# maruchitatsuki/python-based-Sequential-Monte-Carlo-method-with-likelihood-tempering

Measured on AMD Instinct MI355X. Metric: particle-mutation-steps/sec, higher is better.
Workload: dtype f64

## Files before the change

include/smc_hip.h:

```cpp
#ifndef SMC_HIP_H
#define SMC_HIP_H

#include <stddef.h>
#include <stdint.h>

#ifdef __cplusplus
extern "C" {
#endif

#define SMC_ABI_VERSION 3
#define SMC_MAX_DIM 8
#define SMC_MAX_ESS_CAND 16
#define SMC_MAX_RANKS 64

#define SMC_SET_PRED 0
#define SMC_SET_FILT 1

#define SMC_PRIOR_UNIFORM 0
#define SMC_PRIOR_NORMAL 1
#define SMC_PRIOR_FLAT 2
#define SMC_PRIOR_LOGNORMAL 3
#define SMC_PRIOR_GAMMA 4
#define SMC_PRIOR_BETA 5
#define SMC_PRIOR_TRUNCNORMAL 6
// ... 96 lines not shown
int smc_user_model_check4(const char *source, int n_states, int dim, int method, int n_obs, int proportional, char *log, int log_cap);
int smc_user_model_dump_source4(const char *source, int n_states, int dim, int method, int n_obs, int proportional, const char *dir);
int smc_set_model_user5(smc_ctx *ctx, const char *source, int n_states, int n_obs, const double *t, const double *obs,
                        const double *cond, const double *obs_scale, int n_ex, int n_t, int n_cond, const int *add_index,
                        const double *add_fixed, const int *prop_index, const double *prop_fixed, double rtol, double atol, int method,
                        int est_sigma, double sigma_fixed, const double *in_t, const double *in_u, int n_in, int n_knot);
int smc_user_model_check5(const char *source, int n_states, int dim, int method, int n_obs, int noise, int n_cond, int n_in, int n_knot,
                          char *log, int log_cap);
int smc_user_model_dump_source5(const char *source, int n_states, int dim, int method, int n_obs, int noise, int n_cond, int n_in,
                                int n_knot, const char *dir);
int smc_set_model_user6(smc_ctx *ctx, const char *source, int n_states, int n_obs, const double *t, const double *obs,
                        const double *cond, const double *obs_scale, int n_ex, int n_t, int n_cond, const int *add_index,
                        const double *add_fixed, const int *prop_index, const double *prop_fixed, double rtol, double atol, int method,
                        int est_sigma, double sigma_fixed, const double *in_t, const double *in_u, int n_in, int n_knot,
                        const double *ev_t, const double *ev_v, int n_ev, int n_val);
int smc_user_model_check6(const char *source, int n_states, int dim, int method, int n_obs, int noise, int n_cond, int n_in, int n_knot,
                          int n_ev, int n_val, char *log, int log_cap);
int smc_user_model_dump_source6(const char *source, int n_states, int dim, int method, int n_obs, int noise, int n_cond, int n_in,
                                int n_knot, int n_ev, int n_val, const char *dir);
int smc_set_model_user7(smc_ctx *ctx, const char *source, int n_states, int n_obs, const double *t, const double *obs,
                        const double *cond, const double *obs_scale, int n_ex, int n_t, int n_cond, const int *add_index,
                        const double *add_fixed, const int *prop_index, const double *prop_fixed, double rtol, double atol, int method,
                        int est_sigma, double sigma_fixed, const double *in_t, const double *in_u, int n_in, int n_knot,
                        const double *ev_t, const double *ev_v, int n_ev, int n_val, const signed char *censor);
int smc_user_model_check7(const char *source, int n_states, int dim, int method, int n_obs, int noise, int n_cond, int n_in, int n_knot,
                          int n_ev, int n_val, int censor, char *log, int log_cap);
int smc_user_model_dump_source7(const char *source, int n_states, int dim, int method, int n_obs, int noise, int n_cond, int n_in,
                                int n_knot, int n_ev, int n_val, int censor, const char *dir);
int smc_user_predict(smc_ctx *ctx, const double *particle, int64_t n, double *lk, double *pred, int64_t *n_failed, int64_t *attempts);
int smc_user_predict_at(smc_ctx *ctx, const double *particle, int64_t n, const double *t_new, const double *cond_new, int n_ex_new,
                        int n_t_new, double *pred, int64_t *n_failed, int64_t *attempts);
#define SMC_PRED_NOISE_GAUSSIAN 1
#define SMC_PRED_NOISE_FAMILY 2
int smc_user_predict_summary(smc_ctx *ctx, int set, const double *t_new, const double *cond_new, int n_ex_new, int n_t_new,
                             const double *probs, int n_probs, int noise, uint64_t seed, int64_t global_offset,
                             size_t max_staging_bytes, double *mean, double *sd, double *lower, double *upper, int64_t *n_finite,
                             int64_t *n_failed, int64_t *attempts, double *kernel_ms);
int smc_user_pointwise(smc_ctx *ctx, const double *particle, int64_t n, double *ll, int64_t *n_failed, int64_t *attempts);
int smc_user_pointwise_summary(smc_ctx *ctx, int set, size_t max_staging_bytes, int64_t *n, double *max, double *sum_exp, double *mean,
                               double *m2, double *pit, int64_t *n_failed, int64_t *attempts, double *kernel_ms);
typedef struct smc_pointwise_opts {
    int count_pit;
    uint64_t seed;
    int64_t global_offset;
    int64_t *pit_below, *pit_equal, *pit_n;
} smc_pointwise_opts;
int smc_user_pointwise_summary_opt(smc_ctx *ctx, int set, size_t max_staging_bytes, const smc_pointwise_opts *opts, int64_t *n,
                                   double *max, double *sum_exp, double *mean, double *m2, double *pit, int64_t *n_failed,
                                   int64_t *attempts, double *kernel_ms);
int smc_user_sweep_counters(smc_ctx *ctx, int64_t out[4]);
int smc_meth_sweep_counters(smc_ctx *ctx, int64_t out[4]);
int smc_meth_sweep_check(smc_ctx *ctx, int64_t out[5]);
int smc_meth_download_solves(smc_ctx *ctx, double *flows, int32_t *status, int64_t n);
int smc_set_prior(smc_ctx *ctx, const int *kind, const double *a, const double *b, int dim);
int smc_set_prior_ex(smc_ctx *ctx, const int *kind, const double *a, const double *b, const double *lo, const double *hi, int dim);
int smc_prior_check(const int *kind, const double *a, const double *b, const double *lo, const double *hi, int dim);
int smc_set_prior_mode(smc_ctx *ctx, int mode);

#define SMC_RESAMPLE_RESIDUAL_SYSTEMATIC 0
#define SMC_RESAMPLE_SYSTEMATIC 1
#define SMC_RESAMPLE_MULTINOMIAL 2
int smc_set_early_reject(smc_ctx *ctx, int enable);
int smc_set_stiff_first(smc_ctx *ctx, int enable);
int smc_set_cost_order(smc_ctx *ctx, int enable);
int smc_set_fast_tail(smc_ctx *ctx, int enable);
int smc_set_share_replicates(smc_ctx *ctx, int enable);
int smc_mm_group_replicates(const double *t, const double *S0, int n_ex, int n_t, int *primary, int *partner);
int smc_mm_share_info(smc_ctx *ctx, int *n_solve, int64_t *shared_attempts);
int smc_set_start_reject(smc_ctx *ctx, int enable);
int smc_mm_start_reject_info(smc_ctx *ctx, int64_t *not_started);
double smc_mm_reject_threshold(double lk1, double gamma, double rr, double sigma, int n_ex, int n_t, double pratio, int in_support);
int smc_set_in_phase(smc_ctx *ctx, int enable);
int smc_set_exact_pow(smc_ctx *ctx, int enable);
int smc_set_resampling(smc_ctx *ctx, int scheme);

int smc_upload_particles(smc_ctx *ctx, int set, const double *aos, int64_t n);
int smc_download_particles(smc_ctx *ctx, int set, double *aos, int64_t n);
int smc_upload_lk(smc_ctx *ctx, int set, const double *lk, int64_t n);
int smc_download_lk(smc_ctx *ctx, int set, double *lk, int64_t n);
int smc_download_accept_flags(smc_ctx *ctx, uint8_t *flags, int64_t n);
int smc_download_item_info(smc_ctx *ctx, int32_t *info, int64_t n);
int smc_download_item_sums(smc_ctx *ctx, double *sums, int64_t n);
int smc_commit_filt_to_pred(smc_ctx *ctx);
int smc_sample_prior_device(smc_ctx *ctx, uint64_t seed, int64_t global_offset);

int smc_loglik(smc_ctx *ctx, int set, int64_t *n_failed, int64_t *rk_attempts);
int smc_mm_loglik_host(smc_ctx *ctx, const double *particle, int64_t n, double *lk, double *pred, int64_t *n_failed,
                       int64_t *rk_attempts);

int smc_max_lk_local(smc_ctx *ctx, double *max_lk);
int smc_ess_partials(smc_ctx *ctx, double max_lk, const double *gm, int n_cand, double *sum_w, double *sum_w2);
int smc_max_lk_global(smc_ctx *ctx, double *max_lk);
int smc_ess_partials_global(smc_ctx *ctx, double max_lk, const double *gm, int n_cand, double *sum_w, double *sum_w2);
int smc_ess_search_global(smc_ctx *ctx, const double *gm, int n_cand, int with_max, double *max_lk, double *sum_w,
                          double *sum_w2);

int smc_resample_phase1(smc_ctx *ctx, double max_lk, double gm, double sum_weight_global, double *residual_sum_local,
                        int64_t *count_sum_local);
int smc_resample_phase2(smc_ctx *ctx, double max_lk, double gm, double sum_weight_global, double residual_prefix,
                        double wrand, int64_t *offspring_local);
int smc_download_offspring(smc_ctx *ctx, int64_t *p_is, int64_t n);
int smc_resample_phase3(smc_ctx *ctx, const int64_t *out_base_all, const int64_t *offspring_all, int first_step);
int smc_exchange_plan(int world, int rank, int64_t n_local, const int64_t *out_base_all, const int64_t *offspring_all,
                      int64_t *send_off, int64_t *send_cnt, int64_t *src_lo, int64_t *recv_off, int64_t *recv_cnt,
                      int64_t *recv_row, int64_t *own, int64_t *stale_lo);
int smc_resample_global(smc_ctx *ctx, double max_lk, double gm, double sum_weight_global, double wrand, int first_step,
                        int64_t *n_offspring, int64_t *count_sum);

int smc_resample_enqueue(smc_ctx *ctx, double max_lk, double gm, double sum_weight_global, double wrand, int first_step);
int smc_resample_result(smc_ctx *ctx, int64_t *n_offspring, int64_t *count_sum);

int smc_pinned_alloc(size_t bytes, void **out);
int smc_pinned_free(void *p);

int smc_moment_sums_local(smc_ctx *ctx, double *sums);
int smc_moment_centered_local(smc_ctx *ctx, const double *mean, double *centered);

int smc_mh_step_host_rng(smc_ctx *ctx, double gamma, double mhstep_ratio, const double *noise, const double *rr,
                         int64_t n, int64_t *accepted_now, int64_t *accepted_ever, int64_t *n_failed,
                         int64_t *rk_attempts);
int smc_mh_step_device_rng(smc_ctx *ctx, double gamma, double mhstep_ratio, const double *transform, uint64_t seed,
                           uint64_t stream, int64_t global_offset, int64_t *accepted_now, int64_t *accepted_ever,
                           int64_t *n_failed, int64_t *rk_attempts);
int smc_mh_iteration_device_rng(smc_ctx *ctx, double gamma, double mhstep_ratio, const double *w_cov, uint64_t seed,
                                uint64_t stream, int64_t global_offset, int64_t *accepted_now, int64_t *accepted_ever,
                                int64_t *n_failed, int64_t *rk_attempts_local, double *cov_m);
#define SMC_SWEEP_COUNTER_WORDS 14
int smc_mh_sweeps_device_rng(smc_ctx *ctx, double gamma, double mhstep_ratio, const double *w_cov, uint64_t seed,
                             uint64_t stream0, int n_iter, double thr_stop, double thr_halve, int64_t global_offset,
                             int *n_done, int *stopped, double *ratio_next, int64_t *accepted_now, int64_t *accepted_ever,
                             int64_t *n_failed, int64_t *rk_attempts_local, double *ratio_used, double *cov_m,
                             int64_t *sweep_counters);
int smc_proposal_factor_device(smc_ctx *ctx, const double *w_cov, double *cov_m, double *transform);
int smc_mh_iteration_last_transform(smc_ctx *ctx, double *transform);
int smc_reset_accept_flags(smc_ctx *ctx);
int smc_set_debug_capture(smc_ctx *ctx, int enable);
int smc_download_debug_proposals(smc_ctx *ctx, double *aos, double *lk2, uint8_t *p0, uint8_t *r, int64_t n);

int smc_comm_get_unique_id(uint8_t id[128]);
int smc_comm_init(smc_ctx *ctx, const uint8_t id[128], int rank, int world);
int smc_comm_info(smc_ctx *ctx, int *count, int *user_rank, int *device);
int smc_comm_allreduce_sum_f64(smc_ctx *ctx, double *inout, int n);
int smc_comm_allreduce_max_f64(smc_ctx *ctx, double *inout, int n);
int smc_comm_allreduce_sum_i64(smc_ctx *ctx, int64_t *inout, int n);
int smc_comm_allgather_f64(smc_ctx *ctx, const double *in, int n, double *out );
int smc_comm_allgather_i64(smc_ctx *ctx, const int64_t *in, int n, int64_t *out );
int smc_comm_barrier(smc_ctx *ctx);

#ifdef SMC_ENABLE_DEBUG_API
int smc_debug_set_order(smc_ctx *ctx, const int32_t *order, int64_t n, int patience);
int smc_debug_rccl_self_exchange(smc_ctx *ctx, int64_t row, int64_t cnt, int64_t dst_row);
int smc_debug_set_local_peers(smc_ctx *ctx, smc_ctx **peers, int rank, int world);
int smc_resample_phase3_pull(smc_ctx *ctx);
int smc_debug_peer_collectives(smc_ctx *ctx, int enable);
#endif

#define SMC_T_LOGLIK 0
#define SMC_T_MH 1
#define SMC_T_ESS 2
#define SMC_T_RESAMPLE 3
#define SMC_T_MOMENTS 4
#define SMC_T_MAX 5
#define SMC_T_SOLVE 6
#define SMC_T_COUNT 7
int smc_timing_enable(smc_ctx *ctx, int enable);
int smc_timing_reset(smc_ctx *ctx);
// ... 19 lines not shown
```

python-based-sequential-monte-carlo-method-with-likelihood-tempering_amd/binding.py:

```python
from __future__ import annotations

import ctypes
import os
import re

_HERE = os.path.dirname(os.path.abspath(__file__))
LIB_PATH = os.environ.get("SMC_HIP_LIB") or os.path.join(_HERE, "libsmc_hip.so")
HEADER_PATH = os.path.join(os.path.dirname(_HERE), "include", "smc_hip.h")

SMC_SET_PRED, SMC_SET_FILT = 0, 1
SMC_USER_METHOD_RK45, SMC_USER_METHOD_BDF = 0, 1
SMC_USER_MAX_OBS = 8
SMC_USER_MAX_INPUTS, SMC_USER_MAX_KNOTS = 8, 4096
SMC_USER_MAX_EVENTS, SMC_USER_MAX_EVENT_VALUES = 256, 8
SMC_USER_MAX_ROOTS, SMC_USER_MAX_ROOT_FIRES = 4, 256
USER_METHODS = {"RK45": SMC_USER_METHOD_RK45, "BDF": SMC_USER_METHOD_BDF}
SMC_PRIOR_UNIFORM, SMC_PRIOR_NORMAL, SMC_PRIOR_FLAT = 0, 1, 2
SMC_PRIOR_LOGNORMAL, SMC_PRIOR_GAMMA, SMC_PRIOR_BETA, SMC_PRIOR_TRUNCNORMAL = 3, 4, 5, 6
SMC_PRIOR_MODE_MASK, SMC_PRIOR_MODE_RATIO_MASK, SMC_PRIOR_MODE_RATIO = 0, 1, 2
PRIOR_MODES = {"mask": 0, "ratio_mask": 1, "ratio": 2}
RESAMPLING = {"residual_systematic": 0, "systematic": 1, "multinomial": 2}
SMC_MAX_ESS_CAND = 16
SMC_PRED_MAX_PROBS = 16
SMC_PRED_NOISE_GAUSSIAN, SMC_PRED_NOISE_FAMILY = 1, 2
# ... 54 lines not shown
    "smc_device_info": (cint, [c_ctx, ctypes.c_char_p, cint, ctypes.c_char_p, cint, c_ip]),
    "smc_set_model_mm": (cint, [c_ctx, c_dp, c_dp, c_dp, cint, cint, cint, f64, f64, f64]),
    "smc_set_model_methanation": (cint, [c_ctx, c_dp, c_dp, c_dp, cint, c_dp, c_ip, cint, f64, f64, f64, f64]),
    "smc_set_model_user": (cint, [c_ctx, ctypes.c_char_p, cint, c_dp, c_dp, c_dp, cint, cint, cint, cint, f64, f64, f64]),
    "smc_user_model_check": (cint, [ctypes.c_char_p, cint, cint, ctypes.c_char_p, cint]),
    "smc_user_model_dump_source": (cint, [ctypes.c_char_p, cint, cint, ctypes.c_char_p]),
    "smc_set_model_user_spec": (cint, [c_ctx, ctypes.POINTER(UserModelSpec)]),
    "smc_user_model_check_spec": (cint, [ctypes.POINTER(UserSourceSpec), ctypes.c_char_p, cint]),
    "smc_user_model_dump_source_spec": (cint, [ctypes.POINTER(UserSourceSpec), ctypes.c_char_p]),
    "smc_user_spec_layout": (cint, [cint, c_ip, cint]),
    "smc_set_model_user2": (cint, [c_ctx, ctypes.c_char_p, cint, c_dp, c_dp, c_dp, cint, cint, cint, cint, f64, f64, f64, cint]),
    "smc_user_model_check2": (cint, [ctypes.c_char_p, cint, cint, cint, ctypes.c_char_p, cint]),
    "smc_user_model_dump_source2": (cint, [ctypes.c_char_p, cint, cint, cint, ctypes.c_char_p]),
    "smc_set_model_user3": (cint, [c_ctx, ctypes.c_char_p, cint, cint, c_dp, c_dp, c_dp, c_dp, cint, cint, cint, cint, f64, f64, f64,
                                    cint]),
    "smc_user_model_check3": (cint, [ctypes.c_char_p, cint, cint, cint, cint, ctypes.c_char_p, cint]),
    "smc_user_model_dump_source3": (cint, [ctypes.c_char_p, cint, cint, cint, cint, ctypes.c_char_p]),
    "smc_set_model_user4": (cint, [c_ctx, ctypes.c_char_p, cint, cint, c_dp, c_dp, c_dp, c_dp, cint, cint, cint, c_ip, c_dp, c_ip, c_dp,
                                    f64, f64, cint]),
    "smc_user_noise_check": (cint, [cint, cint, c_ip, c_dp, c_ip, c_dp]),
    "smc_user_model_check4": (cint, [ctypes.c_char_p, cint, cint, cint, cint, cint, ctypes.c_char_p, cint]),
    "smc_user_model_dump_source4": (cint, [ctypes.c_char_p, cint, cint, cint, cint, cint, ctypes.c_char_p]),
    "smc_set_model_user5": (cint, [c_ctx, ctypes.c_char_p, cint, cint, c_dp, c_dp, c_dp, c_dp, cint, cint, cint, c_ip, c_dp, c_ip, c_dp,
                                    f64, f64, cint, cint, f64, c_dp, c_dp, cint, cint]),
    "smc_user_input_check": (cint, [c_dp, c_dp, cint, cint, cint]),
    "smc_user_model_check5": (cint, [ctypes.c_char_p, cint, cint, cint, cint, cint, cint, cint, cint, ctypes.c_char_p, cint]),
    "smc_user_model_dump_source5": (cint, [ctypes.c_char_p, cint, cint, cint, cint, cint, cint, cint, cint, ctypes.c_char_p]),
    "smc_user_set_design_inputs": (cint, [c_ctx, c_dp, c_dp, cint, cint]),
    "smc_set_model_user6": (cint, [c_ctx, ctypes.c_char_p, cint, cint, c_dp, c_dp, c_dp, c_dp, cint, cint, cint, c_ip, c_dp, c_ip, c_dp,
                                    f64, f64, cint, cint, f64, c_dp, c_dp, cint, cint, c_dp, c_dp, cint, cint]),
    "smc_user_event_check": (cint, [c_dp, c_dp, c_dp, cint, cint, cint, cint]),
    "smc_user_model_check6": (cint, [ctypes.c_char_p, cint, cint, cint, cint, cint, cint, cint, cint, cint, cint, ctypes.c_char_p, cint]),
    "smc_user_model_dump_source6": (cint, [ctypes.c_char_p, cint, cint, cint, cint, cint, cint, cint, cint, cint, cint, ctypes.c_char_p]),
    "smc_user_set_design_events": (cint, [c_ctx, c_dp, c_dp, cint, cint]),
    "smc_set_model_user7": (cint, [c_ctx, ctypes.c_char_p, cint, cint, c_dp, c_dp, c_dp, c_dp, cint, cint, cint, c_ip, c_dp, c_ip, c_dp,
                                    f64, f64, cint, cint, f64, c_dp, c_dp, cint, cint, c_dp, c_dp, cint, cint, c_i8p]),
    "smc_user_censor_check": (cint, [c_dp, c_dp, c_i8p, cint, cint, cint, cint, cint, cint]),
    "smc_user_obs_family": (cint, [ctypes.c_char_p, c_ip, cint]),
    "smc_user_count_check": (cint, [c_ip, cint, c_dp, c_dp, c_i8p, c_dp, cint, cint, cint, cint, c_ip, c_dp, c_ip, c_dp]),
    "smc_user_model_check7": (cint, [ctypes.c_char_p, cint, cint, cint, cint, cint, cint, cint, cint, cint, cint, cint, ctypes.c_char_p,
                                      cint]),
    "smc_user_model_dump_source7": (cint, [ctypes.c_char_p, cint, cint, cint, cint, cint, cint, cint, cint, cint, cint, cint,
                                            ctypes.c_char_p]),
    "smc_user_predict": (cint, [c_ctx, c_dp, i64, c_dp, c_dp, c_i64p, c_i64p]),
    "smc_user_predict_at": (cint, [c_ctx, c_dp, i64, c_dp, c_dp, cint, cint, c_dp, c_i64p, c_i64p]),
    "smc_user_predict_summary": (cint, [c_ctx, cint, c_dp, c_dp, cint, cint, c_dp, cint, cint, u64, i64, ctypes.c_size_t, c_dp, c_dp,
                                         c_dp, c_dp, c_i64p, c_i64p, c_i64p, c_dp]),
    "smc_user_pointwise": (cint, [c_ctx, c_dp, i64, c_dp, c_i64p, c_i64p]),
    "smc_user_pointwise_summary": (cint, [c_ctx, cint, ctypes.c_size_t, c_i64p, c_dp, c_dp, c_dp, c_dp, c_dp, c_i64p, c_i64p, c_dp]),
    "smc_user_pointwise_summary_opt": (cint, [c_ctx, cint, ctypes.c_size_t, ctypes.POINTER(PointwiseOpts), c_i64p, c_dp, c_dp, c_dp, c_dp,
                                               c_dp, c_i64p, c_i64p, c_dp]),
    "smc_user_sweep_counters": (cint, [c_ctx, c_i64p]),
    "smc_meth_sweep_counters": (cint, [c_ctx, c_i64p]),
    "smc_meth_sweep_check": (cint, [c_ctx, c_i64p]),
    "smc_meth_download_solves": (cint, [c_ctx, c_dp, ctypes.POINTER(ctypes.c_int32), i64]),
    "smc_set_prior": (cint, [c_ctx, c_ip, c_dp, c_dp, cint]),
    "smc_set_prior_ex": (cint, [c_ctx, c_ip, c_dp, c_dp, c_dp, c_dp, cint]),
    "smc_prior_check": (cint, [c_ip, c_dp, c_dp, c_dp, c_dp, cint]),
    "smc_set_prior_mode": (cint, [c_ctx, cint]),
    "smc_set_resampling": (cint, [c_ctx, cint]),
    "smc_set_early_reject": (cint, [c_ctx, cint]),
    "smc_set_stiff_first": (cint, [c_ctx, cint]),
    "smc_set_cost_order": (cint, [c_ctx, cint]),
    "smc_set_fast_tail": (cint, [c_ctx, cint]),
    "smc_set_share_replicates": (cint, [c_ctx, cint]),
    "smc_mm_group_replicates": (cint, [c_dp, c_dp, cint, cint, c_ip, c_ip]),
    "smc_mm_share_info": (cint, [c_ctx, c_ip, c_i64p]),
    "smc_set_start_reject": (cint, [c_ctx, cint]),
    "smc_mm_start_reject_info": (cint, [c_ctx, c_i64p]),
    "smc_mm_reject_threshold": (ctypes.c_double, [ctypes.c_double, ctypes.c_double, ctypes.c_double, ctypes.c_double, cint, cint,
                                                  ctypes.c_double, cint]),
    "smc_set_in_phase": (cint, [c_ctx, cint]),
    "smc_set_exact_pow": (cint, [c_ctx, cint]),
    "smc_exchange_plan": (cint, [cint, cint, i64, c_i64p, c_i64p, c_i64p, c_i64p, c_i64p, c_i64p, c_i64p, c_i64p, c_i64p, c_i64p]),
    "smc_upload_particles": (cint, [c_ctx, cint, c_dp, i64]),
    "smc_download_particles": (cint, [c_ctx, cint, c_dp, i64]),
    "smc_upload_lk": (cint, [c_ctx, cint, c_dp, i64]),
    "smc_download_lk": (cint, [c_ctx, cint, c_dp, i64]),
    "smc_download_accept_flags": (cint, [c_ctx, c_u8p, i64]),
    "smc_download_item_info": (cint, [c_ctx, ctypes.POINTER(ctypes.c_int32), i64]),
    "smc_download_item_sums": (cint, [c_ctx, c_dp, i64]),
    "smc_debug_set_order": (cint, [c_ctx, ctypes.POINTER(ctypes.c_int32), i64, cint]),
    "smc_commit_filt_to_pred": (cint, [c_ctx]),
    "smc_sample_prior_device": (cint, [c_ctx, u64, i64]),
    "smc_loglik": (cint, [c_ctx, cint, c_i64p, c_i64p]),
    "smc_mm_loglik_host": (cint, [c_ctx, c_dp, i64, c_dp, c_dp, c_i64p, c_i64p]),
    "smc_max_lk_local": (cint, [c_ctx, c_dp]),
    "smc_ess_partials": (cint, [c_ctx, f64, c_dp, cint, c_dp, c_dp]),
    "smc_max_lk_global": (cint, [c_ctx, c_dp]),
    "smc_ess_partials_global": (cint, [c_ctx, f64, c_dp, cint, c_dp, c_dp]),
    "smc_ess_search_global": (cint, [c_ctx, c_dp, cint, cint, c_dp, c_dp, c_dp]),
    "smc_resample_global": (cint, [c_ctx, f64, f64, f64, f64, cint, c_i64p, c_i64p]),
    "smc_resample_enqueue": (cint, [c_ctx, f64, f64, f64, f64, cint]),
    "smc_resample_result": (cint, [c_ctx, c_i64p, c_i64p]),
    "smc_pinned_alloc": (cint, [ctypes.c_size_t, ctypes.POINTER(ctypes.c_void_p)]),
    "smc_pinned_free": (cint, [ctypes.c_void_p]),
    "smc_mh_iteration_device_rng": (cint, [c_ctx, f64, f64, c_dp, u64, u64, i64, c_i64p, c_i64p, c_i64p, c_i64p, c_dp]),
    "smc_mh_sweeps_device_rng": (cint, [c_ctx, f64, f64, c_dp, u64, u64, cint, f64, f64, i64, c_ip, c_ip, c_dp, c_i64p, c_i64p,
                                        c_i64p, c_i64p, c_dp, c_dp, c_i64p]),
    "smc_mh_iteration_last_transform": (cint, [c_ctx, c_dp]),
    "smc_proposal_factor_device": (cint, [c_ctx, c_dp, c_dp, c_dp]),
    "smc_resample_phase1": (cint, [c_ctx, f64, f64, f64, c_dp, c_i64p]),
    "smc_resample_phase2": (cint, [c_ctx, f64, f64, f64, f64, f64, c_i64p]),
    "smc_download_offspring": (cint, [c_ctx, c_i64p, i64]),
    "smc_resample_phase3": (cint, [c_ctx, c_i64p, c_i64p, cint]),
    "smc_moment_sums_local": (cint, [c_ctx, c_dp]),
    "smc_moment_centered_local": (cint, [c_ctx, c_dp, c_dp]),
    "smc_mh_step_host_rng": (cint, [c_ctx, f64, f64, c_dp, c_dp, i64, c_i64p, c_i64p, c_i64p, c_i64p]),
    "smc_mh_step_device_rng": (cint, [c_ctx, f64, f64, c_dp, u64, u64, i64, c_i64p, c_i64p, c_i64p, c_i64p]),
    "smc_reset_accept_flags": (cint, [c_ctx]),
    "smc_set_debug_capture": (cint, [c_ctx, cint]),
    "smc_download_debug_proposals": (cint, [c_ctx, c_dp, c_dp, c_u8p, c_u8p, i64]),
    "smc_comm_get_unique_id": (cint, [c_u8p]),
    "smc_comm_init": (cint, [c_ctx, c_u8p, cint, cint]),
    "smc_comm_info": (cint, [c_ctx, c_ip, c_ip, c_ip]),
    "smc_comm_allreduce_sum_f64": (cint, [c_ctx, c_dp, cint]),
    "smc_comm_allreduce_max_f64": (cint, [c_ctx, c_dp, cint]),
    "smc_comm_allreduce_sum_i64": (cint, [c_ctx, c_i64p, cint]),
    "smc_comm_allgather_f64": (cint, [c_ctx, c_dp, cint, c_dp]),
    "smc_comm_allgather_i64": (cint, [c_ctx, c_i64p, cint, c_i64p]),
    "smc_comm_barrier": (cint, [c_ctx]),
    "smc_debug_rccl_self_exchange": (cint, [c_ctx, i64, i64, i64]),
    "smc_debug_set_local_peers": (cint, [c_ctx, ctypes.POINTER(c_ctx), cint, cint]),
    "smc_resample_phase3_pull": (cint, [c_ctx]),
    "smc_debug_peer_collectives": (cint, [c_ctx, cint]),
    "smc_timing_enable": (cint, [c_ctx, cint]),
    "smc_timing_reset": (cint, [c_ctx]),
    "smc_timing_get": (cint, [c_ctx, cint, c_i64p, c_dp]),
    "smc_work_totals": (cint, [c_ctx, c_i64p]),
    "smc_meth_last_error": (ctypes.c_char_p, []),
    "smc_meth_residual_host": (cint, [cint, c_dp, c_dp, c_dp, i64, c_dp]),
    "smc_meth_rate_host": (cint, [cint, c_dp, c_dp, i64, c_dp]),
    "smc_meth_loglike_host": (cint, [cint, c_dp, c_dp, c_dp, i64, cint, c_dp]),
    "smc_meth_dae_host": (cint, [cint, c_dp, c_dp, i64, f64, f64, f64, f64, f64, f64, c_dp, c_dp,
                                 ctypes.POINTER(ctypes.c_int32), c_i64p, c_dp]),
}

_LIB = None


def header_symbols(path: str = HEADER_PATH):
    txt = open(path).read()
    txt = re.sub(r"/\*.*?\*/", "", txt, flags=re.S)
    return sorted(set(re.findall(r"\b(smc_[a-z0-9_]+)\s*\(", txt)) - {"smc_ctx"})


MISSING = set()


def lib():
    global _LIB
    if _LIB is None:
        if not os.path.exists(LIB_PATH):
            raise SmcError(f"{LIB_PATH} is missing: build it with `make -C {os.path.join(_HERE, 'csrc')}` "
                           "(or __graft_entry__.build()); this package has no CPU fallback")
        L = ctypes.CDLL(LIB_PATH)
        for name, (res, args) in SIGNATURES.items():
            try:
                fn = getattr(L, name)
            except AttributeError:
                if not os.environ.get("SMC_HIP_LIB"):
                    raise
                MISSING.add(name)
                continue
            fn.restype = res
            fn.argtypes = args
# ... 12 lines not shown
```

python-based-sequential-monte-carlo-method-with-likelihood-tempering_amd/csrc/smc_api.hip:

```cpp
#include <hip/hip_runtime.h>
#include <rccl/rccl.h>

#include <cmath>
#include <cstddef>
#include <cstdio>
#include <cstdlib>
#include <chrono>
#include <condition_variable>
#include <cstring>
#include <mutex>
#include <new>

#include "exchange_plan.h"
#include "replicate_groups.h"
#include "smc_internal.h"
#include "stage_kernels.h"

using namespace smc;

static thread_local std::string g_err;

#define HIPC(ctx, call)                                                                                   \
    do {                                                                                                  \
        hipError_t e_ = (call);                                                                           \
        if (e_ != hipSuccess) {                                                                           \
            char buf_[512];                                                                               \
            snprintf(buf_, sizeof buf_, "%s failed: %s (%s:%d)", #call, hipGetErrorString(e_), __FILE__,  \
                     __LINE__);                                                                           \
            if (ctx)                                                                                      \
                (ctx)->err = buf_;                                                                        \
            else                                                                                          \
                g_err = buf_;                                                                             \
            return 1;                                                                                     \
        }                                                                                                 \
    } while (0)

#define NCCLC(ctx, call)                                                                                  \
    do {                                                                                                  \
        ncclResult_t e_ = (call);                                                                         \
        if (e_ != ncclSuccess) {                                                                          \
            char buf_[512];                                                                               \
            snprintf(buf_, sizeof buf_, "%s failed: %s (%s:%d)", #call, ncclGetErrorString(e_), __FILE__, \
                     __LINE__);                                                                           \
            if (ctx)                                                                                      \
                (ctx)->err = buf_;                                                                        \
            else                                                                                          \
                g_err = buf_;                                                                             \
            return 1;                                                                                     \
        }                                                                                                 \
    } while (0)

static int fail(smc_ctx *ctx, const char *msg) {
    if (ctx)
        ctx->err = msg;
    else
        g_err = msg;
    return 1;
}
int smc_fail(smc_ctx *ctx, const char *msg) { return fail(ctx, msg); }

namespace smc {
ScopedTimer::ScopedTimer(smc_ctx *ctx, int which) : c(ctx), on(ctx->timing != 0) {
    if (!on) return;
    if (!c->ev_free.empty()) {
        ep = c->ev_free.back();
        c->ev_free.pop_back();
    } else {
        (void)hipEventCreate(&ep.a);
        (void)hipEventCreate(&ep.b);
    }
    ep.which = which;
    (void)hipEventRecord(ep.a, c->stream);
}
ScopedTimer::~ScopedTimer() {
    if (!on) return;
    (void)hipEventRecord(ep.b, c->stream);
    c->ev_used.push_back(ep);
}
}

static void timing_collect(smc_ctx *c) {
    for (auto &ep : c->ev_used) {
        (void)hipEventSynchronize(ep.b);
        float ms = 0.f;
        if (hipEventElapsedTime(&ms, ep.a, ep.b) == hipSuccess) {
            c->t_ms[ep.which] += ms;
            c->t_launches[ep.which] += 1;
        }
        c->ev_free.push_back(ep);
    }
    c->ev_used.clear();
}

static int ensure_item_capacity(smc_ctx *c, int64_t n);
// ... 3 lines not shown
struct PeerBarrier {
    std::mutex m;
    std::condition_variable cv;
    int count = 0;
    unsigned long gen = 0;
};
struct PeerPtrs { const double *p[kPeerMax]; };
__global__ void peer_reduce_kernel(PeerPtrs src, int world, int n, double *out, int is_max) {
    for (int i = blockIdx.x * blockDim.x + threadIdx.x; i < n; i += gridDim.x * blockDim.x) {
        double v = src.p[0][i];
        for (int q = 1; q < world; ++q) v = is_max ? fmax(v, src.p[q][i]) : v + src.p[q][i];
        out[i] = v;
    }
}
__global__ void peer_gather_kernel(PeerPtrs src, int world, int n, double *out) {
    for (int i = blockIdx.x * blockDim.x + threadIdx.x; i < n * world; i += gridDim.x * blockDim.x) out[i] = src.p[i / n][i % n];
}
}
static int peer_host_barrier(smc_ctx *c) {
    PeerBarrier &b = *static_cast<PeerBarrier *>(c->peers[0]->peer_barrier);
    std::unique_lock<std::mutex> lk(b.m);
    const unsigned long g = b.gen;
    if (++b.count == c->world) {
        b.count = 0;
        ++b.gen;
        b.cv.notify_all();
        return 0;
    }
    if (!b.cv.wait_for(lk, std::chrono::seconds(120), [&] { return b.gen != g; }))
        return fail(c, "local-peer collective: a peer did not arrive within 120 s (the ranks disagree on a collective)");
    return 0;
}
static int peer_allreduce(smc_ctx *c, double *buf, size_t n, bool is_max, bool gather, double *gather_out) {
    if (n > (size_t)kPeerWords || (gather && n * c->world > (size_t)kPeerWords)) return fail(c, "local-peer collective: payload too large");
    const int s = c->peer_parity;
    c->peer_parity ^= 1;
    double *slot = c->d_peer_contrib + (size_t)s * kPeerWords;
    HIPC(c, hipMemcpyAsync(slot, buf, n * sizeof(double), hipMemcpyDeviceToDevice, c->stream));
    HIPC(c, hipEventRecord(c->peer_ev[s], c->stream));
    if (peer_host_barrier(c)) return 1;
    PeerPtrs src{};
    for (int q = 0; q < c->world; ++q) {
        src.p[q] = c->peers[q]->d_peer_contrib + (size_t)s * kPeerWords;
        if (q != c->rank) HIPC(c, hipStreamWaitEvent(c->stream, c->peers[q]->peer_ev[s], 0));
    }
    if (gather)
        hipLaunchKernelGGL(peer_gather_kernel, dim3(1), dim3(256), 0, c->stream, src, c->world, (int)n, gather_out);
    else
        hipLaunchKernelGGL(peer_reduce_kernel, dim3(1), dim3(256), 0, c->stream, src, c->world, (int)n, buf, is_max ? 1 : 0);
    HIPC(c, hipGetLastError());
    return 0;
}
static bool peers_on(const smc_ctx *c) { return c->peer_collectives && c->world > 1 && !c->peers.empty(); }
static bool can_reduce(const smc_ctx *c) { return c->nccl_comm != nullptr || peers_on(c); }
static int peer_exchange(smc_ctx *c);

extern "C" {

int smc_abi_version(void) { return SMC_ABI_VERSION; }

const char *smc_last_error(const smc_ctx *ctx) { return ctx ? ctx->err.c_str() : g_err.c_str(); }

int smc_create(smc_ctx **out, int device, int64_t n_local, int64_t n_global, int dim) {
    if (!out) return fail(nullptr, "smc_create: out is NULL");
    *out = nullptr;
    if (n_local <= 0 || n_global < n_local) return fail(nullptr, "smc_create: need 0 < n_local <= n_global");
    if (n_global >= (int64_t)1 << 31) return fail(nullptr, "smc_create: n_global must be < 2^31");
    if (dim < 1 || dim > SMC_MAX_DIM) return fail(nullptr, "smc_create: dim out of range");
    int ndev = 0;
    HIPC((smc_ctx *)nullptr, hipGetDeviceCount(&ndev));
    if (device < 0 || device >= ndev) return fail(nullptr, "smc_create: no such HIP device");
    HIPC((smc_ctx *)nullptr, hipSetDevice(device));
    smc_ctx *c = new (std::nothrow) smc_ctx();
    if (!c) return fail(nullptr, "smc_create: out of host memory");
    c->device = device;
    c->dim = dim;
    c->n_local = n_local;
    c->n_global = n_global;
    {
        const char *e = getenv("SMC_SHARE_REPLICATES");
        c->share_env_off = e ? atoi(e) == 0 : false;
        e = getenv("SMC_START_REJECT");
        c->start_reject_env_off = e ? atoi(e) == 0 : false;
    }
#define CK(call)                                   \
    do {                                           \
        hipError_t e_ = (call);                    \
        if (e_ != hipSuccess) {                    \
            g_err = std::string(#call) + ": " + hipGetErrorString(e_); \
            smc_destroy(c);                        \
            return 1;                              \
        }                                          \
    } while (0)
    CK(hipStreamCreateWithFlags(&c->stream, hipStreamNonBlocking));
    const size_t nb = (size_t)n_local * sizeof(double);
    for (int s = 0; s < 2; ++s) {
        CK(hipMalloc(&c->set[s].theta, nb * dim));
        CK(hipMalloc(&c->set[s].lk, nb));
        CK(hipMemsetAsync(c->set[s].theta, 0, nb * dim, c->stream));
        CK(hipMemsetAsync(c->set[s].lk, 0, nb, c->stream));
        c->set[s].stride = n_local;
    }
    CK(hipMalloc(&c->r_ac, (size_t)n_local));
    CK(hipMemsetAsync(c->r_ac, 0, (size_t)n_local, c->stream));
    CK(hipMalloc(&c->d_counters, sizeof(SweepCounters)));
    CK(hipMalloc(&c->d_queue, 2 * sizeof(unsigned long long)));
    CK(hipMalloc(&c->d_finish_rows, finish_rows_bytes()));
    CK(hipMemsetAsync(c->d_finish_rows, 0, finish_rows_bytes(), c->stream));
    CK(hipMalloc(&c->d_reject, sizeof(RejectArgs)));
    CK(hipMalloc(&c->d_groups, 2 * kMaxEx * sizeof(int)));
    CK(hipMalloc(&c->d_stiff_count, 4 * sizeof(unsigned)));
    CK(hipMemsetAsync(c->d_stiff_count, 0, 4 * sizeof(unsigned), c->stream));
    CK(hipMalloc(&c->d_p0, (size_t)n_local));
    CK(hipMalloc(&c->d_order, (size_t)n_local * sizeof(int32_t)));
    CK(hipMalloc(&c->d_bucket, (size_t)n_local));
    CK(hipMalloc(&c->d_order_hist, cost_table_bytes()));
    CK(hipMemsetAsync(c->d_order_hist, 0, cost_table_bytes(), c->stream));
    CK(hipMalloc(&c->d_sorted, (size_t)n_local * 32));
    {
        hipDeviceProp_t prop;
        CK(hipGetDeviceProperties(&prop, device));
        c->cu_count = prop.multiProcessorCount;
        c->solve_blocks_per_cu = query_solve_blocks_per_cu(false);
        c->solve_blocks_per_cu_fast = query_solve_blocks_per_cu(true);
    }
    CK(hipHostMalloc(&c->h_counters, sizeof(SweepCounters)));
    CK(hipMalloc(&c->d_noise, nb * (dim + 1)));
    c->d_rr = c->d_noise + (size_t)n_local * dim;
    CK(hipMalloc(&c->d_stage, nb * dim));
    c->partials_cap = 2048 * 64;
    CK(hipMalloc(&c->d_partials, (size_t)c->partials_cap * sizeof(double)));
    CK(hipMalloc(&c->d_small, 4096 * sizeof(double)));
    {
        BatchBlock *db = nullptr, *hb = nullptr;
        CK(hipMalloc(&db, sizeof(BatchBlock)));
        c->d_batch = db;
        CK(hipMemsetAsync(db, 0, sizeof(BatchBlock), c->stream));
        CK(hipHostMalloc(&hb, sizeof(BatchBlock)));
        c->h_batch = hb;
        memset(hb, 0, sizeof(BatchBlock));
        c->d_fused = db->fused;  c->h_fused = hb->fused;
        c->d_mhctl = &db->ctl;   c->h_mhctl = &hb->ctl;
        c->d_mhlog = db->log;    c->h_mhlog = hb->log;
    }
    CK(hipMalloc(&c->d_ess, 128 * sizeof(double)));
    CK(hipMemsetAsync(c->d_ess, 0, 128 * sizeof(double), c->stream));
    CK(hipHostMalloc(&c->h_ess, 128 * sizeof(double)));
    CK(hipHostMalloc(&c->h_small, 4096 * sizeof(double)));
    c->n_tiles = (n_local + kScanTile - 1) / kScanTile;
    CK(hipMalloc(&c->d_oscan, (size_t)n_local * sizeof(int32_t)));
    CK(hipMalloc(&c->d_blk_r, (size_t)(c->n_tiles + 1) * sizeof(double)));
    CK(hipMalloc(&c->d_blk_c, (size_t)(c->n_tiles + 1) * sizeof(int64_t)));
    CK(hipMalloc(&c->d_blk_o, (size_t)(c->n_tiles + 1) * sizeof(int64_t)));
    CK(hipMalloc(&c->d_rs, 2 * sizeof(int64_t)));
    CK(hipHostMalloc(&c->h_rs, 2 * sizeof(int64_t)));
    CK(hipStreamSynchronize(c->stream));
#undef CK
    *out = c;
    return 0;
}

void smc_destroy(smc_ctx *c) {
    if (!c) return;
    (void)hipSetDevice(c->device);
    if (c->stream) (void)hipStreamSynchronize(c->stream);
    if (c->nccl_comm) ncclCommDestroy((ncclComm_t)c->nccl_comm);
    for (auto &ep : c->ev_used) {
        (void)hipEventDestroy(ep.a);
        (void)hipEventDestroy(ep.b);
    }
    for (auto &ep : c->ev_free) {
        (void)hipEventDestroy(ep.a);
        (void)hipEventDestroy(ep.b);
    }
    for (int s = 0; s < 2; ++s) {
        (void)hipFree(c->set[s].theta);
        (void)hipFree(c->set[s].lk);
    }
    (void)hipFree(c->r_ac);
    (void)hipFree(c->d_t);
    (void)hipFree(c->d_P);
    (void)hipFree(c->d_S0);
    (void)hipFree(c->d_counters);
    if (c->h_counters) (void)hipHostFree(c->h_counters);
    (void)hipFree(c->d_noise);
    (void)hipFree(c->d_stage);
    (void)hipFree(c->d_partials);
    (void)hipFree(c->d_small);
    (void)hipFree(c->d_batch);
    if (c->h_batch) (void)hipHostFree(c->h_batch);
    (void)hipFree(c->d_ess);
    if (c->h_ess) (void)hipHostFree(c->h_ess);
    if (c->h_small) (void)hipHostFree(c->h_small);
    (void)hipFree(c->d_oscan);
    (void)hipFree(c->d_blk_r);
    (void)hipFree(c->d_blk_c);
    (void)hipFree(c->d_blk_o);
    (void)hipFree(c->d_rs);
    if (c->h_rs) (void)hipHostFree(c->h_rs);
    (void)hipFree(c->d_sendbuf);
    (void)hipFree(c->d_recvbuf);
    (void)hipFree(c->dbg_lk2);
    (void)hipFree(c->dbg_r);
    (void)hipFree(c->d_sum_r2);
    (void)hipFree(c->d_info);
    (void)hipFree(c->d_p0);
    (void)hipFree(c->d_pratio);
    user_model_release(c);
    (void)hipFree(c->d_mn_thr);
    (void)hipFree(c->d_mn_blk);
    (void)hipFree(c->d_queue);
    (void)hipFree(c->d_finish_rows);
    (void)hipFree(c->d_reject);
    (void)hipFree(c->d_groups);
// ... 359 lines not shown
    c->stiff_first = enable != 0;
    return 0;
}

int smc_set_resampling(smc_ctx *c, int scheme) {
    if (!c) return fail(nullptr, "NULL context");
    if (scheme != SMC_RESAMPLE_RESIDUAL_SYSTEMATIC && scheme != SMC_RESAMPLE_SYSTEMATIC && scheme != SMC_RESAMPLE_MULTINOMIAL)
        return fail(c, "Unknown resampling scheme");
    if (scheme == SMC_RESAMPLE_MULTINOMIAL && !c->d_mn_thr) {
        HIPC(c, hipSetDevice(c->device));
        const int64_t m = c->n_global + 1, ntm = (m + kScanTile - 1) / kScanTile;
        HIPC(c, hipMalloc(&c->d_mn_thr, (size_t)m * sizeof(double)));
        HIPC(c, hipMalloc(&c->d_mn_blk, (size_t)(ntm + 1) * sizeof(double)));
    }
    c->resampling = scheme;
    return 0;
}

static int check_set(smc_ctx *c, int set, int64_t n) {
    if (!c) return fail(nullptr, "NULL context");
    if (set != SMC_SET_PRED && set != SMC_SET_FILT) return fail(c, "bad particle set id");
    if (n < 0 || n > c->n_local) return fail(c, "n exceeds the context capacity");
    return 0;
}

int smc_upload_particles(smc_ctx *c, int set, const double *aos, int64_t n) {
    if (check_set(c, set, n)) return 1;
    HIPC(c, hipSetDevice(c->device));
    c->moments_valid = false;
    HIPC(c, hipMemcpyAsync(c->d_stage, aos, (size_t)n * c->dim * sizeof(double), hipMemcpyHostToDevice, c->stream));
    launch_aos_to_soa(c, c->d_stage, c->set[set].theta, n, c->dim, c->set[set].stride);
    HIPC(c, hipStreamSynchronize(c->stream));
    return 0;
}
int smc_download_particles(smc_ctx *c, int set, double *aos, int64_t n) {
    if (check_set(c, set, n)) return 1;
    HIPC(c, hipSetDevice(c->device));
    launch_soa_to_aos(c, c->set[set].theta, c->d_stage, n, c->dim, c->set[set].stride);
    HIPC(c, hipMemcpyAsync(aos, c->d_stage, (size_t)n * c->dim * sizeof(double), hipMemcpyDeviceToHost, c->stream));
    HIPC(c, hipStreamSynchronize(c->stream));
    return 0;
}
int smc_upload_lk(smc_ctx *c, int set, const double *lk, int64_t n) {
    if (check_set(c, set, n)) return 1;
    if (set == SMC_SET_PRED) c->ess_max_valid = false;
    HIPC(c, hipSetDevice(c->device));
    HIPC(c, hipMemcpyAsync(c->set[set].lk, lk, (size_t)n * sizeof(double), hipMemcpyHostToDevice, c->stream));
    HIPC(c, hipStreamSynchronize(c->stream));
    return 0;
}
int smc_download_lk(smc_ctx *c, int set, double *lk, int64_t n) {
    if (check_set(c, set, n)) return 1;
    HIPC(c, hipSetDevice(c->device));
    HIPC(c, hipMemcpyAsync(lk, c->set[set].lk, (size_t)n * sizeof(double), hipMemcpyDeviceToHost, c->stream));
    HIPC(c, hipStreamSynchronize(c->stream));
    return 0;
}
int smc_download_accept_flags(smc_ctx *c, uint8_t *flags, int64_t n) {
    if (check_set(c, SMC_SET_FILT, n)) return 1;
    HIPC(c, hipSetDevice(c->device));
    HIPC(c, hipMemcpyAsync(flags, c->r_ac, (size_t)n, hipMemcpyDeviceToHost, c->stream));
    HIPC(c, hipStreamSynchronize(c->stream));
    return 0;
}
int smc_download_item_info(smc_ctx *c, int32_t *info, int64_t n) {
    if (!c) return fail(nullptr, "NULL context");
    if (c->model_kind != 1 || !c->d_info || n < 0 || n > c->item_cap) return fail(c, "smc_download_item_info: Michaelis-Menten sweeps only, n <= particles of the last sweep");
    HIPC(c, hipSetDevice(c->device));
    HIPC(c, hipMemcpyAsync(info, c->d_info, (size_t)n * c->mm.n_ex * sizeof(int32_t), hipMemcpyDeviceToHost, c->stream));
    HIPC(c, hipStreamSynchronize(c->stream));
    return 0;
}
int smc_download_item_sums(smc_ctx *c, double *sums, int64_t n) {
    if (!c) return fail(nullptr, "NULL context");
    if (c->model_kind != 1 || !c->d_sum_r2 || n < 0 || n > c->item_cap) return fail(c, "smc_download_item_sums: Michaelis-Menten sweeps only, n <= particles of the last sweep");
    HIPC(c, hipSetDevice(c->device));
    HIPC(c, hipMemcpyAsync(sums, c->d_sum_r2, (size_t)n * c->mm.n_ex * sizeof(double), hipMemcpyDeviceToHost, c->stream));
    HIPC(c, hipStreamSynchronize(c->stream));
    return 0;
}
int smc_reset_accept_flags(smc_ctx *c) {
    if (!c) return fail(nullptr, "NULL context");
    HIPC(c, hipSetDevice(c->device));
    HIPC(c, hipMemsetAsync(c->r_ac, 0, (size_t)c->n_local, c->stream));
    return 0;
}
int smc_commit_filt_to_pred(smc_ctx *c) {
    if (!c) return fail(nullptr, "NULL context");
    c->ess_max_valid = false;
    HIPC(c, hipSetDevice(c->device));
    const size_t nb = (size_t)c->n_local * sizeof(double);
    HIPC(c, hipMemcpyAsync(c->set[SMC_SET_PRED].theta, c->set[SMC_SET_FILT].theta, nb * c->dim,
                           hipMemcpyDeviceToDevice, c->stream));
    HIPC(c, hipMemcpyAsync(c->set[SMC_SET_PRED].lk, c->set[SMC_SET_FILT].lk, nb, hipMemcpyDeviceToDevice, c->stream));
    return 0;
}
int smc_sample_prior_device(smc_ctx *c, uint64_t seed, int64_t global_offset) {
    if (!c) return fail(nullptr, "NULL context");
    if (!c->have_prior) return fail(c, "smc_set_prior has not been called");
    HIPC(c, hipSetDevice(c->device));
    launch_sample_prior(c, seed, global_offset);
    HIPC(c, hipGetLastError());
    return 0;
}

static int ensure_item_capacity(smc_ctx *c, int64_t n) {
    if (n <= c->item_cap) return 0;
    HIPC(c, hipStreamSynchronize(c->stream));
    (void)hipFree(c->d_sum_r2);
    (void)hipFree(c->d_info);
    (void)hipFree(c->d_stiff_list);
    c->d_sum_r2 = nullptr;
    c->d_info = nullptr;
    c->d_stiff_list = nullptr;
    c->item_cap = 0;
    HIPC(c, hipMalloc(&c->d_sum_r2, (size_t)n * (c->mm.n_ex + 1) * sizeof(double)));
    HIPC(c, hipMalloc(&c->d_info, (size_t)n * c->mm.n_ex * sizeof(int)));
    HIPC(c, hipMalloc(&c->d_stiff_list, (size_t)n * sizeof(int32_t)));
    HIPC(c, hipMemsetAsync(c->d_stiff_count, 0, 4 * sizeof(unsigned), c->stream));
    c->item_cap = n;
    return 0;
}
static int counters_begin(smc_ctx *c) {
    HIPC(c, hipMemsetAsync(c->d_counters, 0, sizeof(SweepCounters), c->stream));
    return 0;
}
static int counters_end(smc_ctx *c) {
    HIPC(c, hipMemcpyAsync(c->h_counters, c->d_counters, sizeof(SweepCounters), hipMemcpyDeviceToHost, c->stream));
    HIPC(c, hipStreamSynchronize(c->stream));
    if (c->model_kind == 1) {
        c->w_solved_items += (int64_t)c->h_counters->solved_items;
        c->w_rk_attempts += (int64_t)c->h_counters->rk_attempts;
        c->w_not_started += (int64_t)c->h_counters->cancelled_solves;
        c->w_solve_launches += 1;
    }
    if (c->model_kind == 1 && c->pending_sweep_items > 0) {
        c->last_sweep_items = c->pending_sweep_items;
        c->last_sweep_long_items = (int64_t)c->h_counters->long_items;
        if (c->start_look_pending && (int64_t)c->h_counters->cancelled_solves * 100 < c->last_sweep_items) c->start_look_idle = true;
        c->pending_sweep_items = 0;
    }
    if (c->model_kind == 2) {
        const SweepCounters &k = *c->h_counters;
        if (k.completed_solves + k.cancelled_solves != k.expected_solves || k.unsolved_items != 0 || k.wave_split != 0) {
            char buf[320];
            snprintf(buf, sizeof buf, "methanation sweep incomplete: %llu of %llu DAE solves finished (+ %llu cancelled by the exact "
                     "early rejection), %llu live items unsolved, %llu waves split at a dequeue", k.completed_solves,
                     k.expected_solves, k.cancelled_solves, k.unsolved_items, k.wave_split);
            return fail(c, buf);
        }
    }
    return 0;
}

int smc_loglik(smc_ctx *c, int set, int64_t *n_failed, int64_t *rk_attempts) {
    if (check_set(c, set, 0)) return 1;
    if (!c->have_model) return fail(c, "smc_set_model_mm has not been called");
    HIPC(c, hipSetDevice(c->device));
    if (set == SMC_SET_PRED) c->ess_max_valid = false;
    if (counters_begin(c)) return 1;
    {
        ScopedTimer tm(c, SMC_T_LOGLIK);
        if (c->model_kind == 2)
            launch_meth_loglik(c, c->set[set].theta, c->set[set].stride, c->n_local, c->set[set].lk);
        else if (c->model_kind == 3)
            launch_user_loglik(c, c->set[set].theta, c->set[set].stride, c->n_local, c->set[set].lk);
        else
            launch_mm_loglik(c, c->set[set].theta, c->set[set].stride, c->n_local, c->set[set].lk, nullptr);
    }
    HIPC(c, hipGetLastError());
    if (c->launch_failed) { c->launch_failed = false; return 1; }
    if (counters_end(c)) return 1;
    if (n_failed) *n_failed = (int64_t)c->h_counters->n_failed;
    if (rk_attempts) *rk_attempts = (int64_t)c->h_counters->rk_attempts;
    return 0;
}

// ... 67 lines not shown
    HIPC(c, hipSetDevice(c->device));
    {
        ScopedTimer tm(c, SMC_T_ESS);
        launch_ess(c, c->set[SMC_SET_PRED].lk, c->n_local, max_lk, gm, n_cand, c->d_small);
    }
    HIPC(c, hipGetLastError());
    if (fetch_small(c, 2 * ess_padded_k(n_cand))) return 1;
    for (int k = 0; k < n_cand; ++k) {
        sum_w[k] = c->h_small[2 * k];
        sum_w2[k] = c->h_small[2 * k + 1];
    }
    return 0;
}

}
static int dev_allreduce(smc_ctx *c, void *buf, size_t n, ncclDataType_t dt, ncclRedOp_t op) {
    if (!c->nccl_comm) {
        if (peers_on(c)) {
            if (dt != ncclDouble || (op != ncclSum && op != ncclMax)) return fail(c, "local-peer collective: only SUM / MAX of doubles");
            return peer_allreduce(c, static_cast<double *>(buf), n, op == ncclMax, false, nullptr);
        }
        if (c->world > 1) return fail(c, "world > 1 but smc_comm_init has not been called (the *_global entry points need RCCL)");
        return 0;
    }
    NCCLC(c, ncclAllReduce(buf, buf, n, dt, op, (ncclComm_t)c->nccl_comm, c->stream));
    return 0;
}
static int dev_allgather_words(smc_ctx *c, int n) {
    if ((size_t)n * c->world > 2048) return fail(c, "collective payload too large");
    if (!c->nccl_comm && peers_on(c)) {
        if (peer_allreduce(c, c->d_small, (size_t)n, false, true, c->d_small + 2048)) return 1;
        HIPC(c, hipMemcpyAsync(c->h_small, c->d_small + 2048, (size_t)n * c->world * 8, hipMemcpyDeviceToHost, c->stream));
    } else if (!c->nccl_comm) {
        if (c->world > 1) return fail(c, "world > 1 but smc_comm_init has not been called (the *_global entry points need RCCL)");
        HIPC(c, hipMemcpyAsync(c->h_small, c->d_small, (size_t)n * 8, hipMemcpyDeviceToHost, c->stream));
    } else {
        NCCLC(c, ncclAllGather(c->d_small, c->d_small + 2048, (size_t)n, ncclUint64, (ncclComm_t)c->nccl_comm, c->stream));
        HIPC(c, hipMemcpyAsync(c->h_small, c->d_small + 2048, (size_t)n * c->world * 8, hipMemcpyDeviceToHost, c->stream));
    }
    HIPC(c, hipStreamSynchronize(c->stream));
    return 0;
}
extern "C" {

int smc_max_lk_global(smc_ctx *c, double *max_lk) {
    if (!c) return fail(nullptr, "NULL context");
    HIPC(c, hipSetDevice(c->device));
    {
        ScopedTimer tm(c, SMC_T_MAX);
        launch_max(c, c->set[SMC_SET_PRED].lk, c->n_local, c->d_small);
    }
    HIPC(c, hipGetLastError());
    if (dev_allreduce(c, c->d_small, 1, ncclDouble, ncclMax)) return 1;
    if (fetch_small(c, 1)) return 1;
    *max_lk = c->h_small[0];
    return 0;
}

int smc_ess_partials_global(smc_ctx *c, double max_lk, const double *gm, int n_cand, double *sum_w, double *sum_w2) {
    if (!c) return fail(nullptr, "NULL context");
    if (n_cand < 1 || n_cand > SMC_MAX_ESS_CAND) return fail(c, "n_cand out of range");
    HIPC(c, hipSetDevice(c->device));
    {
        ScopedTimer tm(c, SMC_T_ESS);
        launch_ess(c, c->set[SMC_SET_PRED].lk, c->n_local, max_lk, gm, n_cand, c->d_small);
    }
    HIPC(c, hipGetLastError());
    const int nv = 2 * ess_padded_k(n_cand);
    if (dev_allreduce(c, c->d_small, (size_t)nv, ncclDouble, ncclSum)) return 1;
    if (fetch_small(c, nv)) return 1;
    for (int k = 0; k < n_cand; ++k) {
        sum_w[k] = c->h_small[2 * k];
        sum_w2[k] = c->h_small[2 * k + 1];
    }
    return 0;
}

int smc_ess_search_global(smc_ctx *c, const double *gm, int n_cand, int with_max, double *max_lk, double *sum_w, double *sum_w2) {
    if (!c) return fail(nullptr, "NULL context");
    if (n_cand < 1 || n_cand > 2 * SMC_MAX_ESS_CAND) return fail(c, "smc_ess_search_global: n_cand must be 1 .. 32");
    HIPC(c, hipSetDevice(c->device));
    constexpr int kMaxAt = 0, kSumsAt = 8;
    double *S = c->d_ess;
    if (with_max) {
        {
            ScopedTimer tm(c, SMC_T_MAX);
            launch_max(c, c->set[SMC_SET_PRED].lk, c->n_local, S + kMaxAt);
        }
        if (dev_allreduce(c, S + kMaxAt, 1, ncclDouble, ncclMax)) return 1;
        c->ess_max_valid = true;
    } else if (!c->ess_max_valid) {
        return fail(c, "smc_ess_search_global: with_max == 0 needs an earlier call with with_max != 0 on the same lk");
    }
    const int n_a = n_cand < SMC_MAX_ESS_CAND ? n_cand : SMC_MAX_ESS_CAND, n_b = n_cand - n_a;
    const int pad_a = ess_padded_k(n_a), pad_b = n_b > 0 ? ess_padded_k(n_b) : 0;
    {
        ScopedTimer tm(c, SMC_T_ESS);
        launch_ess(c, c->set[SMC_SET_PRED].lk, c->n_local, 0.0, gm, n_a, S + kSumsAt, S + kMaxAt);
        if (n_b > 0) launch_ess(c, c->set[SMC_SET_PRED].lk, c->n_local, 0.0, gm + n_a, n_b, S + kSumsAt + 2 * pad_a, S + kMaxAt);
    }
    HIPC(c, hipGetLastError());
    const int nv = 2 * (pad_a + pad_b);
    if (dev_allreduce(c, S + kSumsAt, (size_t)nv, ncclDouble, ncclSum)) return 1;
    HIPC(c, hipMemcpyAsync(c->h_ess + kMaxAt, S + kMaxAt, (size_t)(kSumsAt - kMaxAt + nv) * sizeof(double), hipMemcpyDeviceToHost,
                           c->stream));
    HIPC(c, hipStreamSynchronize(c->stream));
    if (max_lk) *max_lk = c->h_ess[kMaxAt];
    for (int k = 0; k < n_cand; ++k) {
        const int at = kSumsAt + (k < n_a ? 2 * k : 2 * pad_a + 2 * (k - n_a));
        sum_w[k] = c->h_ess[at];
        sum_w2[k] = c->h_ess[at + 1];
    }
    return 0;
}

int smc_resample_global(smc_ctx *c, double max_lk, double gm, double sum_weight_global, double wrand, int first_step,
                        int64_t *n_offspring, int64_t *count_sum) {
    if (!c) return fail(nullptr, "NULL context");
    HIPC(c, hipSetDevice(c->device));
    const int W = c->world, R = c->rank;
    {
        ScopedTimer tm(c, SMC_T_RESAMPLE);
        launch_resample_phase1(c, max_lk, gm, sum_weight_global);
        HIPC(c, hipMemcpyAsync(c->d_small, c->d_blk_r + c->n_tiles, 8, hipMemcpyDeviceToDevice, c->stream));
        HIPC(c, hipMemcpyAsync(c->d_small + 1, c->d_blk_c + c->n_tiles, 8, hipMemcpyDeviceToDevice, c->stream));
    }
    HIPC(c, hipGetLastError());
    if (dev_allgather_words(c, 2)) return 1;
    double prefix = 0.0;
    int64_t csum = 0;
    for (int q = 0; q < W; ++q) {
        int64_t cq;
        memcpy(&cq, c->h_small + 2 * q + 1, sizeof cq);
        csum += cq;
        if (q < R) prefix = prefix + c->h_small[2 * q];
    }
    {
        ScopedTimer tm(c, SMC_T_RESAMPLE);
        launch_resample_phase2(c, max_lk, gm, sum_weight_global, prefix, wrand);
        HIPC(c, hipMemcpyAsync(c->d_small, c->d_blk_o + c->n_tiles, 8, hipMemcpyDeviceToDevice, c->stream));
    }
    HIPC(c, hipGetLastError());
    if (dev_allgather_words(c, 1)) return 1;
    std::vector<int64_t> o_all(W), bases(W);
    int64_t tot = 0;
    for (int q = 0; q < W; ++q) {
        memcpy(&o_all[q], c->h_small + q, sizeof(int64_t));
        bases[q] = tot;
        tot += o_all[q];
    }
    if (smc_resample_phase3(c, bases.data(), o_all.data(), first_step)) return 1;
    if (n_offspring) *n_offspring = tot;
    if (count_sum) *count_sum = csum;
    return 0;
}

int smc_resample_enqueue(smc_ctx *c, double max_lk, double gm, double sum_weight_global, double wrand, int first_step) {
    if (!c) return fail(nullptr, "NULL context");
    HIPC(c, hipSetDevice(c->device));
    if (c->world > 1) {
        int64_t o = 0, cs = 0;
        if (smc_resample_global(c, max_lk, gm, sum_weight_global, wrand, first_step, &o, &cs)) return 1;
        c->h_rs[0] = cs;
        c->h_rs[1] = o;
        c->rs_pending = 2;
        return 0;
    }
    c->moments_valid = false;
    {
        ScopedTimer tm(c, SMC_T_RESAMPLE);
        launch_resample_phase1(c, max_lk, gm, sum_weight_global);
        launch_resample_phase2(c, max_lk, gm, sum_weight_global, 0.0, wrand);
        launch_resample_gather_all(c, first_step, c->d_rs);
    }
    HIPC(c, hipGetLastError());
    HIPC(c, hipMemcpyAsync(c->h_rs, c->d_rs, 2 * sizeof(int64_t), hipMemcpyDeviceToHost, c->stream));
    c->rs_pending = 1;
    return 0;
}
int smc_resample_result(smc_ctx *c, int64_t *n_offspring, int64_t *count_sum) {
    if (!c) return fail(nullptr, "NULL context");
    if (!c->rs_pending) return fail(c, "smc_resample_result: no smc_resample_enqueue before it");
    HIPC(c, hipSetDevice(c->device));
    if (c->rs_pending == 1) HIPC(c, hipStreamSynchronize(c->stream));
    c->rs_pending = 0;
    if (count_sum) *count_sum = c->h_rs[0];
    if (n_offspring) *n_offspring = c->h_rs[1];
    if (c->h_rs[1] > c->n_global)
        return fail(c, "resampling produced more offspring than particles (the reference raises IndexError, "
                       "Micmem_SMC_main.py:180)");
    return 0;
}

int smc_pinned_alloc(size_t bytes, void **out) {
    if (!out || bytes == 0) return fail(nullptr, "smc_pinned_alloc: bad arguments");
    *out = nullptr;
    HIPC((smc_ctx *)nullptr, hipHostMalloc(out, bytes));
    return 0;
}
int smc_pinned_free(void *p) {
    if (p) HIPC((smc_ctx *)nullptr, hipHostFree(p));
    return 0;
}

int smc_resample_phase1(smc_ctx *c, double max_lk, double gm, double sum_weight_global, double *residual_sum_local,
                        int64_t *count_sum_local) {
    if (!c) return fail(nullptr, "NULL context");
    HIPC(c, hipSetDevice(c->device));
    {
        ScopedTimer tm(c, SMC_T_RESAMPLE);
        launch_resample_phase1(c, max_lk, gm, sum_weight_global);
    }
    HIPC(c, hipGetLastError());
    HIPC(c, hipMemcpyAsync(c->h_small, c->d_blk_r + c->n_tiles, sizeof(double), hipMemcpyDeviceToHost, c->stream));
    HIPC(c, hipMemcpyAsync(c->h_small + 1, c->d_blk_c + c->n_tiles, sizeof(int64_t), hipMemcpyDeviceToHost, c->stream));
    HIPC(c, hipStreamSynchronize(c->stream));
    *residual_sum_local = c->h_small[0];
    int64_t cs;
    memcpy(&cs, c->h_small + 1, sizeof cs);
    *count_sum_local = cs;
    return 0;
}

int smc_resample_phase2(smc_ctx *c, double max_lk, double gm, double sum_weight_global, double residual_prefix,
                        double wrand, int64_t *offspring_local) {
    if (!c) return fail(nullptr, "NULL context");
    HIPC(c, hipSetDevice(c->device));
    {
        ScopedTimer tm(c, SMC_T_RESAMPLE);
        launch_resample_phase2(c, max_lk, gm, sum_weight_global, residual_prefix, wrand);
    }
    HIPC(c, hipGetLastError());
    HIPC(c, hipMemcpyAsync(c->h_small, c->d_blk_o + c->n_tiles, sizeof(int64_t), hipMemcpyDeviceToHost, c->stream));
    HIPC(c, hipStreamSynchronize(c->stream));
    int64_t o;
    memcpy(&o, c->h_small, sizeof o);
    *offspring_local = o;
    return 0;
}

int smc_download_offspring(smc_ctx *c, int64_t *p_is, int64_t n) {
    if (check_set(c, SMC_SET_PRED, n)) return 1;
    HIPC(c, hipSetDevice(c->device));
    int64_t *d_tmp = nullptr;
    HIPC(c, hipMalloc(&d_tmp, (size_t)c->n_local * sizeof(int64_t)));
    launch_offspring_from_scan(c, d_tmp);
    hipError_t e = hipMemcpyAsync(p_is, d_tmp, (size_t)n * sizeof(int64_t), hipMemcpyDeviceToHost, c->stream);
    if (e == hipSuccess) e = hipStreamSynchronize(c->stream);
    (void)hipFree(d_tmp);
    HIPC(c, e);
    return 0;
}
// ... 192 lines not shown
        HIPC(c, hipEventCreateWithFlags(&c->peer_pull_ev, hipEventDisableTiming));
        c->peer_barrier = new (std::nothrow) PeerBarrier();
        if (!c->peer_barrier) return fail(c, "out of memory");
    }
    c->peer_collectives = enable != 0;
    return 0;
}

int smc_resample_phase3_pull(smc_ctx *c) {
    if (!c) return fail(nullptr, "NULL context");
    if (c->peers.empty()) return fail(c, "smc_debug_set_local_peers has not been called");
    HIPC(c, hipSetDevice(c->device));
    c->moments_valid = false;
    if (peer_pull_copies(c)) return 1;
    HIPC(c, hipStreamSynchronize(c->stream));
    return 0;
}

int smc_moment_sums_local(smc_ctx *c, double *sums) {
    if (!c) return fail(nullptr, "NULL context");
    HIPC(c, hipSetDevice(c->device));
    {
        ScopedTimer tm(c, SMC_T_MOMENTS);
        launch_moment_sums(c, c->d_small);
    }
    HIPC(c, hipGetLastError());
    if (fetch_small(c, c->dim)) return 1;
    for (int i = 0; i < c->dim; ++i) sums[i] = c->h_small[i];
    return 0;
}
int smc_moment_centered_local(smc_ctx *c, const double *mean, double *centered) {
    if (!c) return fail(nullptr, "NULL context");
    HIPC(c, hipSetDevice(c->device));
    {
        ScopedTimer tm(c, SMC_T_MOMENTS);
        launch_moment_centered(c, mean, c->d_small);
    }
    HIPC(c, hipGetLastError());
    const int d = c->dim;
    if (fetch_small(c, d * (d + 1) / 2)) return 1;
    int k = 0;
    for (int a = 0; a < d; ++a)
        for (int b = a; b < d; ++b) {
            centered[a * d + b] = c->h_small[k];
            centered[b * d + a] = c->h_small[k];
            ++k;
        }
    return 0;
}

static int mh_finish(smc_ctx *c, int64_t *accepted_now, int64_t *accepted_ever, int64_t *n_failed, int64_t *rk_attempts) {
    HIPC(c, hipGetLastError());
    if (c->launch_failed) { c->launch_failed = false; return 1; }
    if (counters_end(c)) return 1;
    if (accepted_now) *accepted_now = (int64_t)c->h_counters->accepted_now;
    if (accepted_ever) *accepted_ever = (int64_t)c->h_counters->accepted_ever;
    if (n_failed) *n_failed = (int64_t)c->h_counters->n_failed;
    if (rk_attempts) *rk_attempts = (int64_t)c->h_counters->rk_attempts;
    return 0;
}

int smc_mh_step_host_rng(smc_ctx *c, double gamma, double mhstep_ratio, const double *noise, const double *rr, int64_t n,
                         int64_t *accepted_now, int64_t *accepted_ever, int64_t *n_failed, int64_t *rk_attempts) {
    if (!c) return fail(nullptr, "NULL context");
    if (!c->have_model || !c->have_prior) return fail(c, "model and prior must be set before an MH step");
    if (n != c->n_local) return fail(c, "smc_mh_step_host_rng: n must equal the context's n_local");
    HIPC(c, hipSetDevice(c->device));
    c->moments_valid = false;
    const int d = c->dim;
    HIPC(c, hipMemcpyAsync(c->d_stage, noise, (size_t)n * d * sizeof(double), hipMemcpyHostToDevice, c->stream));
    launch_aos_to_soa(c, c->d_stage, c->d_noise, n, d, n);
    HIPC(c, hipMemcpyAsync(c->d_rr, rr, (size_t)n * sizeof(double), hipMemcpyHostToDevice, c->stream));
    if (counters_begin(c)) return 1;
    MHParams mh{};
    mh.gamma = gamma;
    mh.ratio = mhstep_ratio;
    mh.noise = c->d_noise;
    mh.rr = c->d_rr;
    mh.device_rng = 0;
    mh.prior_mode = c->prior_mode;
    mh.pratio = c->d_pratio;
    {
        ScopedTimer tm(c, SMC_T_MH);
        if (c->model_kind == 2) launch_meth_mh(c, n, mh); else if (c->model_kind == 3) launch_user_mh(c, n, mh); else launch_mm_mh(c, n, mh);
    }
    return mh_finish(c, accepted_now, accepted_ever, n_failed, rk_attempts);
}

int smc_mh_step_device_rng(smc_ctx *c, double gamma, double mhstep_ratio, const double *transform, uint64_t seed,
                           uint64_t stream, int64_t global_offset, int64_t *accepted_now, int64_t *accepted_ever,
                           int64_t *n_failed, int64_t *rk_attempts) {
    if (!c) return fail(nullptr, "NULL context");
    if (!c->have_model || !c->have_prior) return fail(c, "model and prior must be set before an MH step");
    HIPC(c, hipSetDevice(c->device));
    c->moments_valid = false;
    if (counters_begin(c)) return 1;
    MHParams mh{};
    mh.gamma = gamma;
    mh.ratio = mhstep_ratio;
    mh.device_rng = 1;
    mh.prior_mode = c->prior_mode;
    mh.pratio = c->d_pratio;
    mh.seed = seed;
    mh.stream = stream;
    mh.global_offset = global_offset;
    for (int i = 0; i < c->dim * c->dim; ++i) mh.transform[i] = transform[i];
    {
        ScopedTimer tm(c, SMC_T_MH);
        if (c->model_kind == 2) launch_meth_mh(c, c->n_local, mh); else if (c->model_kind == 3) launch_user_mh(c, c->n_local, mh); else launch_mm_mh(c, c->n_local, mh);
    }
    return mh_finish(c, accepted_now, accepted_ever, n_failed, rk_attempts);
}

constexpr int kV = 0;
constexpr int kSums = 64;
constexpr int kCent = 72;
constexpr int kShift = 112;
constexpr int kCov = 128;
constexpr int kXf = 192;
constexpr int kFusedWords = 256;

static int two_pass_factor(smc_ctx *c, const double *w_cov) {
    const int d = c->dim, npair = d * (d + 1) / 2;
    double *S = c->d_fused;
    ScopedTimer tm(c, SMC_T_MOMENTS);
    launch_moment_sums(c, S + kSums);
    if (dev_allreduce(c, S + kSums, (size_t)d, ncclDouble, ncclSum)) return 1;
    launch_moment_centered_dev(c, S + kSums, S + kCent);
    if (dev_allreduce(c, S + kCent, (size_t)npair, ncclDouble, ncclSum)) return 1;
    launch_mh_transform(c, S + kCent, S + kSums, w_cov, S + kShift, S + kCov, S + kXf);
    return 0;
}

int smc_mh_iteration_device_rng(smc_ctx *c, double gamma, double mhstep_ratio, const double *w_cov, uint64_t seed,
                                uint64_t stream, int64_t global_offset, int64_t *accepted_now, int64_t *accepted_ever,
                                int64_t *n_failed, int64_t *rk_attempts_local, double *cov_m) {
    if (!c) return fail(nullptr, "NULL context");
    if (!c->have_model || !c->have_prior) return fail(c, "model and prior must be set before an MH step");
    if (!w_cov) return fail(c, "smc_mh_iteration_device_rng: w_cov is NULL");
    HIPC(c, hipSetDevice(c->device));
    const int d = c->dim;
    const bool mm = c->model_kind == 1;
    double *S = c->d_fused;
    if (mm && c->moments_valid) {
        ScopedTimer tm(c, SMC_T_MOMENTS);
        launch_mh_transform(c, S + kV, nullptr, w_cov, S + kShift, S + kCov, S + kXf);
    } else if (two_pass_factor(c, w_cov)) {
        return 1;
    }
    c->moments_valid = false;
    MHParams mh{};
    mh.gamma = gamma;
    mh.ratio = mhstep_ratio;
    mh.device_rng = 1;
    mh.prior_mode = c->prior_mode;
    mh.pratio = c->d_pratio;
    mh.seed = seed;
    mh.stream = stream;
    mh.global_offset = global_offset;
    mh.transform_dev = S + kXf;
    if (mm) {
        mh.zero_counters = c->d_counters;
        mh.zero_queue = c->d_queue;
        mh.moment_shift = S + kShift;
        mh.moment_rows = c->d_partials;
    } else if (counters_begin(c)) {
        return 1;
    }
    {
        ScopedTimer tm(c, SMC_T_MH);
        if (c->model_kind == 2) launch_meth_mh(c, c->n_local, mh); else if (c->model_kind == 3) launch_user_mh(c, c->n_local, mh); else launch_mm_mh(c, c->n_local, mh);
    }
    HIPC(c, hipGetLastError());
    if (c->launch_failed) { c->launch_failed = false; return 1; }
    const int nv = mm ? d + d * (d + 1) / 2 : 0;
    launch_moments_reduce(c, mm ? c->moment_rows_n : 0, nv, S + kV);
    if (dev_allreduce(c, S + kV, (size_t)nv + 3, ncclDouble, ncclSum)) return 1;
    HIPC(c, hipMemcpyAsync(c->h_fused, S, (size_t)kFusedWords * sizeof(double), hipMemcpyDeviceToHost, c->stream));
    if (counters_end(c)) return 1;
    c->moments_valid = mm;
    if (accepted_now) *accepted_now = (int64_t)c->h_fused[kV + nv];
    if (accepted_ever) *accepted_ever = (int64_t)c->h_fused[kV + nv + 1];
    if (n_failed) *n_failed = (int64_t)c->h_fused[kV + nv + 2];
    if (rk_attempts_local) *rk_attempts_local = (int64_t)c->h_counters->rk_attempts;
    if (cov_m)
        for (int i = 0; i < d * d; ++i) cov_m[i] = c->h_fused[kCov + i];
    return 0;
}

int smc_mh_sweeps_device_rng(smc_ctx *c, double gamma, double mhstep_ratio, const double *w_cov, uint64_t seed, uint64_t stream0,
                             int n_iter, double thr_stop, double thr_halve, int64_t global_offset, int *n_done, int *stopped,
                             double *ratio_next, int64_t *accepted_now, int64_t *accepted_ever, int64_t *n_failed,
                             int64_t *rk_attempts_local, double *ratio_used, double *cov_m, int64_t *sweep_counters) {
    if (!c) return fail(nullptr, "NULL context");
    if (!c->have_model || !c->have_prior) return fail(c, "model and prior must be set before an MH step");
    if (c->model_kind != 1 && c->model_kind != 2)
        return fail(c, "smc_mh_sweeps_device_rng: Michaelis-Menten and methanation models (a user model takes smc_mh_iteration_device_rng)");
    if (!w_cov) return fail(c, "smc_mh_sweeps_device_rng: w_cov is NULL");
    if (n_iter < 1 || n_iter > kMHBatchMax) return fail(c, "smc_mh_sweeps_device_rng: n_iter must be 1 .. 32");
    if (c->world > 1 && !can_reduce(c)) return fail(c, "world > 1 but smc_comm_init has not been called (the batch needs RCCL)");
    HIPC(c, hipSetDevice(c->device));
    const bool mm = c->model_kind == 1;
    const int d = c->dim, npair = d * (d + 1) / 2;
    const int nv = mm ? d + npair : 0;
    const bool one_rank = !can_reduce(c);
    const bool fuse_ctl = mm && one_rank && d == 3;
    double *S = c->d_fused;
    double *vec = mm ? S + kV : S + kCent + npair;
    MHControlArgs a{};
    a.ctl = c->d_mhctl;
    a.log = c->d_mhlog;
    a.ratio0 = mhstep_ratio;
    a.thr_stop = thr_stop;
    a.thr_halve = thr_halve;
    a.nv = nv;
    a.vec = vec;
    a.counters = c->d_counters;
    a.n_global = (double)c->n_global;
    a.shift_io = S + kShift;
    a.cov_out = S + kCov;
    a.xform_out = S + kXf;
    const int parity0 = c->stiff_parity;
    auto bail = [&]() {
        (void)hipStreamSynchronize(c->stream);
        c->stiff_parity = parity0;
        c->moments_valid = false;
        return 1;
    };
    auto two_pass = [&](int extra) {
        launch_moment_sums(c, S + kSums);
        if (dev_allreduce(c, S + kSums, (size_t)d, ncclDouble, ncclSum)) return 1;
        launch_moment_centered_dev(c, S + kSums, S + kCent);
        return dev_allreduce(c, S + kCent, (size_t)(npair + extra), ncclDouble, ncclSum);
    };
    ScopedTimer tm_mh(c, SMC_T_MH);
    {
        ScopedTimer tm(c, SMC_T_MOMENTS);
        a.mode = kCtlInit | kCtlTransform;
        a.iteration = 0;
        if (mm && c->moments_valid) {
            a.mom = S + kV;
            a.sums = nullptr;
        } else {
            if (two_pass(0)) return bail();
            a.mom = S + kCent;
            a.sums = S + kSums;
        }
        launch_mh_control(c, a, w_cov);
    }
    c->moments_valid = false;
    for (int i = 0; i < n_iter; ++i) {
        MHParams mh{};
        mh.gamma = gamma;
        mh.ratio = mhstep_ratio;
        mh.device_rng = 1;
        mh.prior_mode = c->prior_mode;
        mh.pratio = c->d_pratio;
        mh.seed = seed;
        mh.stream = stream0 + (uint64_t)i;
        mh.global_offset = global_offset;
        mh.transform_dev = S + kXf;
        mh.zero_counters = c->d_counters;
        mh.ctl = c->d_mhctl;
        if (mm) {
            mh.zero_queue = c->d_queue;
            mh.moment_shift = S + kShift;
            mh.moment_rows = c->d_partials;
            if (fuse_ctl) {
                a.counts_local = 0;
                a.mom = S + kV;
                a.sums = nullptr;
                a.mode = kCtlDecide | (i + 1 < n_iter ? kCtlTransform : 0);
                a.iteration = i + 1;
            }
            launch_mm_mh(c, c->n_local, mh, fuse_ctl ? &a : nullptr, w_cov);
        } else {
            launch_meth_mh(c, c->n_local, mh);
        }
        if (hipGetLastError() != hipSuccess) { fail(c, "smc_mh_sweeps_device_rng: a kernel launch of the batch failed"); return bail(); }
        if (c->launch_failed) { c->launch_failed = false; return bail(); }
        if (fuse_ctl) continue;
        const bool transform_next = i + 1 < n_iter;
        ScopedTimer tm(c, SMC_T_MOMENTS);
        if (mm) {
            if (!one_rank) {
                launch_moments_reduce(c, c->moment_rows_n, nv, vec, c->d_mhctl);
                if (dev_allreduce(c, vec, (size_t)nv + 3, ncclDouble, ncclSum)) return bail();
            }
            a.rows = one_rank ? c->d_partials : nullptr;
            a.n_rows = c->moment_rows_n;
            a.counts_local = 0;
            a.mom = S + kV;
            a.sums = nullptr;
        } else {
            a.rows = nullptr;
            a.n_rows = 0;
            a.counts_local = one_rank ? 1 : 0;
            if (!one_rank) launch_moments_reduce(c, 0, 0, vec, c->d_mhctl);
            if (transform_next) {
                if (two_pass(one_rank ? 0 : 3)) return bail();
            } else if (!one_rank && dev_allreduce(c, vec, 3, ncclDouble, ncclSum)) {
                return bail();
            }
            a.mom = S + kCent;
            a.sums = S + kSums;
        }
        a.mode = kCtlDecide | (transform_next ? kCtlTransform : 0);
        a.iteration = i + 1;
        launch_mh_control(c, a, w_cov);
    }
    if (hipGetLastError() != hipSuccess) { fail(c, "smc_mh_sweeps_device_rng: a kernel launch of the batch failed"); return bail(); }
    HIPC(c, hipMemcpyAsync(c->h_batch, c->d_batch, offsetof(BatchBlock, log) + (size_t)(n_iter + 1) * sizeof(MHLogEntry),
                           hipMemcpyDeviceToHost, c->stream));
    HIPC(c, hipStreamSynchronize(c->stream));
    const int done = c->h_mhctl->n_done;
    if (done < 1 || done > n_iter) return fail(c, "smc_mh_sweeps_device_rng: the device reports an impossible iteration count");
    c->moments_valid = mm;
    *c->h_counters = c->h_mhlog[done - 1].snap;
    if (mm) {
        c->stiff_parity = parity0 ^ (done & 1);
        c->pending_sweep_items = 0;
        c->last_sweep_items = c->n_local * c->mm.n_ex;
        c->last_sweep_long_items = (int64_t)c->h_mhlog[done - 1].long_items;
        if (c->start_look_pending && (int64_t)c->h_mhlog[done - 1].snap.cancelled_solves * 100 < c->last_sweep_items) c->start_look_idle = true;
        c->w_solve_launches += done;
        c->w_noop_launches += n_iter - done;
    }
    if (n_done) *n_done = done;
    if (stopped) *stopped = c->h_mhctl->stop;
    if (ratio_next) *ratio_next = c->h_mhctl->ratio;
    static_assert(sizeof(SweepCounters) == SMC_SWEEP_COUNTER_WORDS * sizeof(unsigned long long), "include/smc_hip.h: SMC_SWEEP_COUNTER_WORDS");
    for (int i = 0; i < done; ++i) {
        const MHLogEntry &e = c->h_mhlog[i];
// ... 200 lines not shown
```

python-based-sequential-monte-carlo-method-with-likelihood-tempering_amd/csrc/smc_internal.h:

```cpp
#pragma once
#include <hip/hip_runtime.h>
#include <stdint.h>

#include <string>
#include <vector>

#include "../../include/smc_hip.h"
#include "sweep_args.h"

int smc_fail(smc_ctx *ctx, const char *msg);

namespace smc {

constexpr int kWave = 64;
constexpr int kMaxEx = 16;
constexpr int kMaxNt = 256;
constexpr int kScanBlock = 256;
constexpr int kScanItems = 4;
constexpr int kScanTile = kScanBlock * kScanItems;

struct MMModel {
    const double *t;
    const double *P_obs;
    const double *S0;
// ... 150 lines not shown
    int device = 0;
    int dim = 0;
    int64_t n_local = 0, n_global = 0;
    hipStream_t stream = nullptr;
    std::string err;

    smc::ParticleSet set[2]{};
    uint8_t *r_ac = nullptr;

    int model_kind = 0;
    void *user = nullptr;
    bool launch_failed = false;
    smc::MethModel meth{};
    double *d_mcond = nullptr, *d_mguess = nullptr, *d_mobs = nullptr, *d_mflows = nullptr, *d_mlk2 = nullptr;
    int *d_mstatus = nullptr;
    int64_t *d_mwork = nullptr;
    double *d_mstat = nullptr;
    int *d_morder = nullptr;
    bool have_model = false, have_prior = false;
    smc::MMModel mm{};
    double *d_t = nullptr, *d_P = nullptr, *d_S0 = nullptr;
    smc::Prior prior{};

    smc::SweepCounters *d_counters = nullptr;
    smc::SweepCounters *h_counters = nullptr;
    double *d_noise = nullptr, *d_rr = nullptr;
    double *d_stage = nullptr;
    double *d_partials = nullptr;
    int64_t partials_cap = 0;
    double *d_small = nullptr, *h_small = nullptr;
    smc::BatchBlock *d_batch = nullptr, *h_batch = nullptr;
    double *d_fused = nullptr, *h_fused = nullptr;
    double *d_ess = nullptr, *h_ess = nullptr;
    bool ess_max_valid = false;
    smc::MHControl *d_mhctl = nullptr;
    smc::MHLogEntry *d_mhlog = nullptr, *h_mhlog = nullptr;
    smc::MHControl *h_mhctl = nullptr;
    int32_t *d_oscan = nullptr;
    double *d_blk_r = nullptr;
    int64_t *d_blk_c = nullptr;
    int64_t *d_blk_o = nullptr;
    int64_t *d_rs = nullptr, *h_rs = nullptr;
    int rs_pending = 0;
    int64_t n_tiles = 0;
    double *d_sendbuf = nullptr;
    int64_t sendbuf_cap = 0;
    double *d_recvbuf = nullptr;
    int64_t recvbuf_cap = 0;
    double *d_sum_r2 = nullptr;
    int *d_info = nullptr;
    int64_t item_cap = 0;
    uint8_t *d_p0 = nullptr;
    double *d_pratio = nullptr;
    int prior_mode = 0;
    int resampling = 0;
    int early_reject = 1;
    double *d_mn_thr = nullptr;
    double *d_mn_blk = nullptr;
    unsigned long long *d_queue = nullptr;
    unsigned long long *d_finish_rows = nullptr;
    smc::RejectArgs *d_reject = nullptr;
    int start_reject = 1;
    bool start_reject_env_off = false;
    bool start_look_pending = false, start_look_idle = false;
    int64_t w_not_started = 0;
    int32_t *d_stiff_list = nullptr;
    unsigned *d_stiff_count = nullptr;
    int stiff_parity = 0;
    int32_t *d_order = nullptr;
    uint8_t *d_bucket = nullptr;
    unsigned *d_order_hist = nullptr;
    void *d_sorted = nullptr;
    int cost_order = 1;
    int order_debug = 0, order_debug_patience = 0;
    int fast_tail = 1;
    int stiff_first = 1;
    int in_phase = 1;
    int64_t last_sweep_items = 0, last_sweep_long_items = 0, pending_sweep_items = 0;
    int share_replicates = 1;
    bool share_env_off = false;
    int n_solve = 0, partner_mask = 0;
    int groups[2 * smc::kMaxEx]{};
    int *d_groups = nullptr;
    int exact_pow = 0;
    bool solve_lds_raised = false;
    int cu_count = 0, solve_blocks_per_cu = 0, solve_blocks_per_cu_fast = 0;
    int debug_capture = 0;
    double *dbg_lk2 = nullptr;
    uint8_t *dbg_r = nullptr;
    double *d_hb_theta = nullptr, *d_hb_lk = nullptr, *d_hb_pred = nullptr;
    int64_t hb_cap = 0, hb_pred_cap = 0;
    bool moments_valid = false;
    int moment_rows_n = 0;

    void *nccl_comm = nullptr;
    int rank = 0, world = 1;
    std::vector<smc_ctx *> peers;
    std::vector<int64_t> plan_send_off, plan_send_cnt, plan_base, plan_cnt;
    bool peer_collectives = false;
    double *d_peer_contrib = nullptr;
    hipEvent_t peer_ev[2]{};
    hipEvent_t peer_pack_ev = nullptr, peer_pull_ev = nullptr;
    bool peer_pull_recorded = false;
    int peer_parity = 0;
    void *peer_barrier = nullptr;

    int timing = 0;
    std::vector<smc::EventPair> ev_used;
    std::vector<smc::EventPair> ev_free;
    int64_t t_launches[SMC_T_COUNT]{};
    double t_ms[SMC_T_COUNT]{};
    int64_t w_solved_items = 0, w_rk_attempts = 0, w_solve_launches = 0, w_noop_launches = 0;
};

namespace smc {

void launch_mm_loglik(smc_ctx *ctx, const double *theta, int64_t stride, int64_t n, double *lk, double *pred);
void launch_mm_mh(smc_ctx *ctx, int64_t n, const MHParams &mh, const MHControlArgs *ctl_after = nullptr, const double *w_cov = nullptr);
size_t finish_rows_bytes();
int solves_per_particle(const smc_ctx *ctx);
unsigned long long *finish_shared_attempts(const smc_ctx *ctx);
int query_solve_blocks_per_cu(bool fast);
constexpr int kInPhasePatience = 12;
size_t cost_table_bytes();
const unsigned *cost_n_ordered(const smc_ctx *ctx);
const unsigned *launch_cost_sort_order(smc_ctx *ctx, int64_t n);
void launch_meth_loglik(smc_ctx *ctx, const double *theta, int64_t stride, int64_t n, double *lk);
void launch_meth_mh(smc_ctx *ctx, int64_t n, const MHParams &mh);
void launch_generic_propose(smc_ctx *ctx, int64_t n, const MHParams &mh);
void launch_generic_accept(smc_ctx *ctx, int64_t n, const MHParams &mh, const double *lk2);
void launch_user_loglik(smc_ctx *ctx, const double *theta, int64_t stride, int64_t n, double *lk);
void launch_user_mh(smc_ctx *ctx, int64_t n, const MHParams &mh);
void user_model_release(smc_ctx *ctx);

struct ScopedTimer {
    smc_ctx *c;
    EventPair ep{};
    bool on;
    ScopedTimer(smc_ctx *ctx, int which);
    ~ScopedTimer();
};

}
```

python-based-sequential-monte-carlo-method-with-likelihood-tempering_amd/csrc/stage_kernels.h:

```cpp
#pragma once
#include "smc_internal.h"

namespace smc {
void launch_aos_to_soa(smc_ctx *c, const double *aos, double *soa, int64_t n, int d, int64_t stride);
void launch_soa_to_aos(smc_ctx *c, const double *soa, double *aos, int64_t n, int d, int64_t stride);
void launch_sample_prior(smc_ctx *c, uint64_t seed, int64_t goff);
void launch_max(smc_ctx *c, const double *lk, int64_t n, double *d_out);
void launch_ess(smc_ctx *c, const double *lk, int64_t n, double max_lk, const double *gm, int k, double *d_out,
                const double *max_lk_dev = nullptr);
int ess_padded_k(int k);
void launch_moment_sums(smc_ctx *c, double *d_out);
void launch_moment_centered(smc_ctx *c, const double *mean, double *d_out);
void launch_moment_centered_dev(smc_ctx *c, const double *d_sums, double *d_out);
void launch_mh_transform(smc_ctx *c, const double *d_mom, const double *d_sums, const double *w_cov, double *d_shift,
                         double *d_cov, double *d_xform);
void launch_moments_reduce(smc_ctx *c, int n_rows, int nv, double *d_out, const MHControl *ctl = nullptr);
void launch_mh_control(smc_ctx *c, const MHControlArgs &a, const double *w_cov);
void launch_resample_phase1(smc_ctx *c, double max_lk, double gm, double sum_w);
void launch_resample_phase2(smc_ctx *c, double max_lk, double gm, double sum_w, double base, double wrand);
void launch_offspring_from_scan(smc_ctx *c, int64_t *d_out);
void launch_resample_gather(smc_ctx *c, int64_t m_lo, int64_t m_hi, double *dst_theta, int64_t dst_stride,
                            double *dst_lk, int64_t dst_off);
void launch_resample_stale(smc_ctx *c, int64_t lo, int64_t hi, int first_step);
void launch_resample_gather_all(smc_ctx *c, int first_step, int64_t *d_result);
}
```

python-based-sequential-monte-carlo-method-with-likelihood-tempering_amd/csrc/stage_kernels.hip:

```cpp
#include <hip/hip_runtime.h>

#include <cstdlib>

#include <cstring>

#include "mh_control.h"
#include "philox.h"
#include "prior_draw.h"
#include "smc_internal.h"
#include "stage_kernels.h"

namespace smc {

__device__ __forceinline__ double wave_max(double v) {
#pragma unroll
    for (int off = 32; off > 0; off >>= 1) {
        const double o = __shfl_down(v, off);
        v = (o > v || o != o) ? o : v;
    }
    return v;
}

template <typename T>
__device__ __forceinline__ T block_sum(T v, T *lds ) {
// ... 5 lines not shown
    T r = lds[0];
    for (int i = 1; i < (int)(blockDim.x >> 6); ++i) r += lds[i];
    return r;
}

template <typename T>
__device__ __forceinline__ T block_inclusive_scan(T v, T *lds , T *total) {
    const int w = threadIdx.x >> 6, l = threadIdx.x & 63;
#pragma unroll
    for (int off = 1; off < 64; off <<= 1) {
        const T o = __shfl_up(v, off);
        if (l >= off) v += o;
    }
    __syncthreads();
    if (l == 63) lds[w] = v;
    __syncthreads();
    T base = 0;
    T tot = 0;
    for (int i = 0; i < (int)(blockDim.x >> 6); ++i) {
        if (i < w) base += lds[i];
        tot += lds[i];
    }
    *total = tot;
    return v + base;
}

__global__ void aos_to_soa_kernel(const double *__restrict__ aos, double *__restrict__ soa, int64_t n, int d,
                                  int64_t stride) {
    const int64_t i = (int64_t)blockIdx.x * blockDim.x + threadIdx.x;
    if (i >= n * d) return;
    const int64_t p = i / d;
    const int c = (int)(i - p * d);
    soa[c * stride + p] = aos[i];
}
__global__ void soa_to_aos_kernel(const double *__restrict__ soa, double *__restrict__ aos, int64_t n, int d,
                                  int64_t stride) {
    const int64_t i = (int64_t)blockIdx.x * blockDim.x + threadIdx.x;
    if (i >= n * d) return;
    const int64_t p = i / d;
    const int c = (int)(i - p * d);
    aos[i] = soa[c * stride + p];
}

__global__ void sample_prior_kernel(Prior prior, double *__restrict__ theta, int64_t stride, int64_t n, uint64_t seed,
                                    int64_t goff) {
    const int64_t p = (int64_t)blockIdx.x * blockDim.x + threadIdx.x;
    if (p >= n) return;
    const uint64_t g = (uint64_t)(goff + p);
    for (int c = 0; c < prior.d; ++c) {
        if (prior.n_new && prior.kind[c] >= SMC_PRIOR_LOGNORMAL) {
            theta[c * stride + p] = smc_draw::prior_draw(prior.kind[c], prior.a[c], prior.b[c], prior.lo[c], prior.hi[c], seed, g, (uint64_t)c);
            continue;
        }
        const u32x4 r = philox_block(seed, g, 0xFFFFFFFF00000000ull | (uint64_t)c, 0);
        double v;
        if (prior.kind[c] == SMC_PRIOR_UNIFORM) {
            v = prior.a[c] + (prior.b[c] - prior.a[c]) * u01_from(r.x, r.y);
        } else {
            const double u1 = 1.0 - u01_from(r.x, r.y), u2 = u01_from(r.z, r.w);
            v = prior.a[c] + prior.b[c] * (sqrt(-2.0 * log(u1)) * cos(6.283185307179586 * u2));
        }
        theta[c * stride + p] = v;
    }
}

__global__ void __launch_bounds__(kScanBlock) max_partial_kernel(const double *__restrict__ lk, int64_t n,
                                                                 double *__restrict__ partials) {
    __shared__ double lds[4];
    double m = -__longlong_as_double(0x7ff0000000000000LL);
    for (int64_t i = (int64_t)blockIdx.x * blockDim.x + threadIdx.x; i < n; i += (int64_t)gridDim.x * blockDim.x) {
        const double v = lk[i];
        m = (v > m || v != v) ? v : m;
    }
    m = wave_max(m);
    const int w = threadIdx.x >> 6, l = threadIdx.x & 63;
    if (l == 0) lds[w] = m;
    __syncthreads();
    if (threadIdx.x == 0) {
        double r = lds[0];
        for (int i = 1; i < 4; ++i) r = (lds[i] > r || lds[i] != lds[i]) ? lds[i] : r;
        partials[blockIdx.x] = r;
    }
}
__global__ void __launch_bounds__(kScanBlock) max_final_kernel(const double *__restrict__ partials, int np,
                                                               double *__restrict__ out) {
    __shared__ double lds[4];
    double m = -__longlong_as_double(0x7ff0000000000000LL);
    for (int i = threadIdx.x; i < np; i += blockDim.x) {
        const double v = partials[i];
        m = (v > m || v != v) ? v : m;
    }
    m = wave_max(m);
    const int w = threadIdx.x >> 6, l = threadIdx.x & 63;
    if (l == 0) lds[w] = m;
    __syncthreads();
    if (threadIdx.x == 0) {
        double r = lds[0];
        for (int i = 1; i < 4; ++i) r = (lds[i] > r || lds[i] != lds[i]) ? lds[i] : r;
        out[0] = r;
    }
}

struct EssCand {
    double gm[SMC_MAX_ESS_CAND];
    int k;
};

template <int NV, int CNT, int OFF>
struct WaveSumStep {
    static __device__ __forceinline__ void run(double (&v)[NV], int lane) {
        if constexpr (CNT > 1) {
            constexpr int half = CNT / 2;
            const bool upper = (lane & OFF) != 0;
#pragma unroll
            for (int i = 0; i < half; ++i) {
                const double keep = upper ? v[i + half] : v[i];
                const double give = upper ? v[i] : v[i + half];
                v[i] = keep + __shfl_xor(give, OFF);
            }
        } else {
            v[0] += __shfl_xor(v[0], OFF);
        }
        if constexpr (OFF > 1) WaveSumStep<NV, (CNT > 1 ? CNT / 2 : 1), OFF / 2>::run(v, lane);
    }
};
template <int NV>
__device__ __forceinline__ void wave_sum_transposed(double (&v)[NV], int lane) {
    static_assert(NV >= 1 && NV <= 64 && (NV & (NV - 1)) == 0, "NV must be a power of two");
    WaveSumStep<NV, NV, 32>::run(v, lane);
}

template <int K>
__global__ void __launch_bounds__(kScanBlock) ess_partial_kernel(const double *__restrict__ lk, int64_t n, double max_lk_val,
                                                                 const double *__restrict__ max_lk_dev, EssCand cand,
                                                                 double *__restrict__ partials) {
    const double max_lk = max_lk_dev ? *max_lk_dev : max_lk_val;
    constexpr int NV = 2 * K;
    constexpr int kShift = NV == 2 ? 5 : NV == 8 ? 3 : NV == 16 ? 2 : 1;
    static_assert(NV == 2 || NV == 8 || NV == 16 || NV == 32, "K must be 1, 4, 8 or 16");
    __shared__ double s_part[kScanBlock / 64][NV];
    double v[NV];
#pragma unroll
    for (int k = 0; k < NV; ++k) v[k] = 0.0;
    for (int64_t i = (int64_t)blockIdx.x * blockDim.x + threadIdx.x; i < n; i += (int64_t)gridDim.x * blockDim.x) {
        const double d = lk[i] - max_lk;
#pragma unroll
        for (int k = 0; k < K; ++k) {
            const double w = exp(d * cand.gm[k]);
            v[2 * k] += w;
            v[2 * k + 1] += w * w;
        }
    }
    const int lane = threadIdx.x & 63, wave = threadIdx.x >> 6;
    wave_sum_transposed<NV>(v, lane);
    if ((lane & ((1 << kShift) - 1)) == 0) s_part[wave][lane >> kShift] = v[0];
    __syncthreads();
    if (threadIdx.x < NV) {
        double r = s_part[0][threadIdx.x];
        for (int w = 1; w < (int)(blockDim.x >> 6); ++w) r += s_part[w][threadIdx.x];
        partials[(size_t)blockIdx.x * NV + threadIdx.x] = r;
    }
}
__global__ void __launch_bounds__(kScanBlock) sum_rows_final_kernel(const double *__restrict__ partials, int np,
                                                                    int nvals, double *__restrict__ out) {
    __shared__ double lds[4];
    for (int v = blockIdx.x; v < nvals; v += gridDim.x) {
        double s = 0.0;
        for (int i = threadIdx.x; i < np; i += blockDim.x) s += partials[(size_t)i * nvals + v];
        s = block_sum(s, lds);
        if (threadIdx.x == 0) out[v] = s;
    }
}

__global__ void __launch_bounds__(kScanBlock) moment_sum_kernel(const double *__restrict__ theta, int64_t stride,
                                                                int64_t n, int d, double *__restrict__ partials) {
    __shared__ double lds[4];
    for (int c = 0; c < d; ++c) {
        double s = 0.0;
        const double *x = theta + c * stride;
        for (int64_t i = (int64_t)blockIdx.x * blockDim.x + threadIdx.x; i < n; i += (int64_t)gridDim.x * blockDim.x)
            s += x[i];
        s = block_sum(s, lds);
        if (threadIdx.x == 0) partials[(size_t)blockIdx.x * d + c] = s;
    }
}
struct MeanArg {
    double m[SMC_MAX_DIM];
};
__global__ void __launch_bounds__(kScanBlock) moment_centered_kernel(const double *__restrict__ theta, int64_t stride,
                                                                     int64_t n, int d, MeanArg mean,
                                                                     const double *__restrict__ dev_sums, double n_div,
                                                                     double *__restrict__ partials) {
    __shared__ double lds[4];
    __shared__ double s_mu[SMC_MAX_DIM];
    double acc[SMC_MAX_DIM * (SMC_MAX_DIM + 1) / 2];
    const int npair = d * (d + 1) / 2;
    if ((int)threadIdx.x < d) s_mu[threadIdx.x] = dev_sums ? dev_sums[threadIdx.x] / n_div : mean.m[threadIdx.x];
    __syncthreads();
    for (int k = 0; k < npair; ++k) acc[k] = 0.0;
    for (int64_t i = (int64_t)blockIdx.x * blockDim.x + threadIdx.x; i < n; i += (int64_t)gridDim.x * blockDim.x) {
        double x[SMC_MAX_DIM];
        for (int c = 0; c < d; ++c) x[c] = theta[c * stride + i] - s_mu[c];
        int k = 0;
        for (int a = 0; a < d; ++a)
            for (int b = a; b < d; ++b) acc[k++] += x[a] * x[b];
    }
    for (int k = 0; k < npair; ++k) {
        const double s = block_sum(acc[k], lds);
        if (threadIdx.x == 0) partials[(size_t)blockIdx.x * npair + k] = s;
    }
}

template <int D>
__global__ void mh_transform_kernel(const double *__restrict__ mom, const double *__restrict__ sums, double n_global, WCov wcov,
                                    double *__restrict__ shift_io, double *__restrict__ cov_out,
                                    double *__restrict__ xform_out) {
    if (threadIdx.x != 0 || blockIdx.x != 0) return;
    mh_transform_body<D>(mom, sums, n_global, wcov, shift_io, cov_out, xform_out);
}

template <int D>
__global__ void __launch_bounds__(kScanBlock) mh_control_kernel(MHControlArgs a, WCov wcov) {
    __shared__ double wpart[kScanBlock / 64][D + D * (D + 1) / 2];
    mh_control_body<D, false>(a, wcov, wpart);
}

struct ResampleArgs {
    double max_lk, gm, sum_w;
    double n_global, inv_np;
    double wrand, base;
    int first_rank;
    int scheme;
    const double *thr;
    int64_t n_thr;
    double s_full;
};

__device__ __forceinline__ void resample_item(const ResampleArgs &a, double lk, double &resid, int64_t &cnt) {
    const double w = exp((lk - a.max_lk) * a.gm) / a.sum_w;
    if (a.scheme != SMC_RESAMPLE_RESIDUAL_SYSTEMATIC) {
        cnt = 0;
        resid = w;
        return;
    }
    const double c = trunc(w * a.n_global);
    cnt = (int64_t)c;
    resid = w - c * a.inv_np;
}

__global__ void __launch_bounds__(kScanBlock) resample_tile_sums_kernel(const double *__restrict__ lk, int64_t n,
                                                                        ResampleArgs a, double *__restrict__ blk_r,
                                                                        int64_t *__restrict__ blk_c) {
    __shared__ double lds_d[4];
    __shared__ int64_t lds_i[4];
    const int64_t base = ((int64_t)blockIdx.x * kScanBlock + threadIdx.x) * kScanItems;
    double rs = 0.0;
    int64_t cs = 0;
#pragma unroll
    for (int k = 0; k < kScanItems; ++k) {
        const int64_t i = base + k;
        if (i < n) {
            double r;
            int64_t c;
            resample_item(a, lk[i], r, c);
            rs += r;
            cs += c;
        }
    }
    rs = block_sum(rs, lds_d);
    cs = block_sum(cs, lds_i);
    if (threadIdx.x == 0) {
        blk_r[blockIdx.x] = rs;
        blk_c[blockIdx.x] = cs;
    }
}

template <typename T>
__global__ void __launch_bounds__(kScanBlock) tile_exclusive_scan_kernel(T *__restrict__ v, int64_t nt) {
    __shared__ T lds[4];
    const int64_t chunk = (nt + kScanBlock - 1) / kScanBlock;
    const int64_t lo = (int64_t)threadIdx.x * chunk, hi = (lo + chunk < nt) ? lo + chunk : nt;
    T s = 0;
    for (int64_t i = lo; i < hi; ++i) s += v[i];
    T total;
    const T incl = block_inclusive_scan(s, lds, &total);
    T run = incl - s;
    for (int64_t i = lo; i < hi; ++i) {
        const T x = v[i];
        v[i] = run;
        run += x;
    }
    if (threadIdx.x == 0) v[nt] = total;
}

__device__ __forceinline__ int64_t thresholds_below(double S, const ResampleArgs &a) {
    if (a.scheme == SMC_RESAMPLE_RESIDUAL_SYSTEMATIC)
        return (S >= a.wrand) ? (int64_t)floor((S - a.wrand) * a.n_global) + 1 : 0;
    if (!(S > 0.0)) return 0;
    if (S >= a.s_full) return a.n_thr;
    int64_t m;
    if (a.scheme == SMC_RESAMPLE_MULTINOMIAL) {
        int64_t lo = 0, hi = a.n_thr;
        while (lo < hi) {
            const int64_t mid = (lo + hi) >> 1;
            if (a.thr[mid] <= S) lo = mid + 1; else hi = mid;
        }
// ... 35 lines not shown
    }
    double tile_total;
    const double incl = block_inclusive_scan(s, lds, &tile_total);
    double run = blk_excl[blockIdx.x] + (incl - s);
    const double inv_total = 1.0 / blk_excl[nt];
#pragma unroll
    for (int k = 0; k < kScanItems; ++k) {
        const int64_t i = base + k;
        run += e[k];
        if (i < m) thr[i] = run * inv_total;
    }
}

__global__ void __launch_bounds__(kScanBlock)
resample_offspring_kernel(const double *__restrict__ lk, int64_t n, ResampleArgs a, const double *__restrict__ blk_r_excl,
                          int32_t *__restrict__ oscan, int64_t *__restrict__ blk_o) {
    __shared__ double lds_d[4];
    __shared__ int64_t lds_i[4];
    __shared__ double thread_start[kScanBlock + 1];
    const int64_t base = ((int64_t)blockIdx.x * kScanBlock + threadIdx.x) * kScanItems;
    double r[kScanItems];
    int64_t c[kScanItems];
    double rs = 0.0;
#pragma unroll
    for (int k = 0; k < kScanItems; ++k) {
        const int64_t i = base + k;
        r[k] = 0.0;
        c[k] = 0;
        if (i < n) resample_item(a, lk[i], r[k], c[k]);
        rs += r[k];
    }
    double tile_total;
    const double incl = block_inclusive_scan(rs, lds_d, &tile_total);
    const double tile_start = a.base + blk_r_excl[blockIdx.x];
    const double tile_end = a.base + blk_r_excl[blockIdx.x + 1];
    thread_start[threadIdx.x] = tile_start + (incl - rs);
    if (threadIdx.x == 0) thread_start[kScanBlock] = tile_end;
    __syncthreads();
    double S = thread_start[threadIdx.x];
    const double S_end = thread_start[threadIdx.x + 1];
    int64_t m_prev = thresholds_below(S, a);
    if (a.first_rank && blockIdx.x == 0 && threadIdx.x == 0) m_prev = 0;
    int64_t o[kScanItems];
    int64_t os = 0;
#pragma unroll
    for (int k = 0; k < kScanItems; ++k) {
        const int64_t i = base + k;
        o[k] = 0;
        if (i < n) {
            const bool last = (k == kScanItems - 1);
            S = (i + 1 >= n) ? tile_end : (last ? S_end : S + r[k]);
            const int64_t m = thresholds_below(S, a);
            int64_t extra = m - m_prev;
            if (extra < 0) extra = 0;
            m_prev = (m > m_prev) ? m : m_prev;
            o[k] = c[k] + extra;
            os += o[k];
        }
    }
    int64_t tile_o;
    const int64_t incl_o = block_inclusive_scan(os, lds_i, &tile_o);
    int64_t run = incl_o - os;
#pragma unroll
    for (int k = 0; k < kScanItems; ++k) {
        const int64_t i = base + k;
        if (i < n) {
            run += o[k];
            oscan[i] = (int32_t)run;
        }
    }
    if (threadIdx.x == 0) blk_o[blockIdx.x] = tile_o;
}

__global__ void __launch_bounds__(kScanBlock) resample_apply_prefix_kernel(int32_t *__restrict__ oscan, int64_t n,
                                                                           const int64_t *__restrict__ blk_o_excl) {
    const int64_t base = ((int64_t)blockIdx.x * kScanBlock + threadIdx.x) * kScanItems;
    const int32_t off = (int32_t)blk_o_excl[blockIdx.x];
#pragma unroll
    for (int k = 0; k < kScanItems; ++k) {
        const int64_t i = base + k;
        if (i < n) oscan[i] += off;
    }
}

__global__ void offspring_from_scan_kernel(const int32_t *__restrict__ oscan, int64_t n, int64_t *__restrict__ p_is) {
    const int64_t i = (int64_t)blockIdx.x * blockDim.x + threadIdx.x;
    if (i >= n) return;
    p_is[i] = (int64_t)oscan[i] - (i ? (int64_t)oscan[i - 1] : 0);
}

__global__ void __launch_bounds__(256)
resample_gather_kernel(const int32_t *__restrict__ oscan, int64_t n, const double *__restrict__ src_theta,
                       int64_t src_stride, const double *__restrict__ src_lk, int d, int64_t m_lo, int64_t m_hi,
                       double *__restrict__ dst_theta, int64_t dst_stride, double *__restrict__ dst_lk, int64_t dst_off) {
    const int64_t k = (int64_t)blockIdx.x * blockDim.x + threadIdx.x;
    const int64_t m = m_lo + k;
    if (m >= m_hi) return;
    int64_t lo = 0, hi = n;
    while (lo < hi) {
        const int64_t mid = (lo + hi) >> 1;
        if ((int64_t)oscan[mid] > m)
            hi = mid;
        else
            lo = mid + 1;
    }
    const int64_t j = lo;
    for (int c = 0; c < d; ++c) dst_theta[c * dst_stride + dst_off + k] = src_theta[c * src_stride + j];
    dst_lk[dst_off + k] = src_lk[j];
}

__global__ void __launch_bounds__(256)
resample_gather_all_kernel(const int32_t *__restrict__ oscan, int64_t n, const double *__restrict__ src_theta, int64_t src_stride,
                           const double *__restrict__ src_lk, int d, const int64_t *__restrict__ count_total,
                           const int64_t *__restrict__ offspring_total, int first_step, double *__restrict__ dst_theta,
                           int64_t dst_stride, double *__restrict__ dst_lk, int64_t *__restrict__ result ) {
    const int64_t m = (int64_t)blockIdx.x * blockDim.x + threadIdx.x;
    const int64_t total = *offspring_total;
    if (m == 0) {
        result[0] = *count_total;
        result[1] = total;
    }
    if (m >= n) return;
    if (m < total) {
        int64_t lo = 0, hi = n;
        while (lo < hi) {
            const int64_t mid = (lo + hi) >> 1;
            if ((int64_t)oscan[mid] > m)
                hi = mid;
            else
                lo = mid + 1;
        }
        const int64_t j = lo < n ? lo : n - 1;
        for (int c = 0; c < d; ++c) dst_theta[c * dst_stride + m] = src_theta[c * src_stride + j];
        dst_lk[m] = src_lk[j];
    } else {
        for (int c = 0; c < d; ++c) dst_theta[c * dst_stride + m] = first_step ? 0.0 : src_theta[c * src_stride + m];
        dst_lk[m] = first_step ? 0.0 : src_lk[m];
    }
}

__global__ void resample_stale_rows_kernel(const double *__restrict__ src_theta, int64_t src_stride,
                                           const double *__restrict__ src_lk, int d, int64_t lo, int64_t hi,
                                           int first_step, double *__restrict__ dst_theta, int64_t dst_stride,
                                           double *__restrict__ dst_lk) {
    const int64_t i = lo + (int64_t)blockIdx.x * blockDim.x + threadIdx.x;
    if (i >= hi) return;
    for (int c = 0; c < d; ++c) dst_theta[c * dst_stride + i] = first_step ? 0.0 : src_theta[c * src_stride + i];
    dst_lk[i] = first_step ? 0.0 : src_lk[i];
}

static inline int reduce_grid(int64_t n, int cap = 2048) {
    static const int ess_cap = [] {
        const char *e = getenv("SMC_REDUCE_BLOCKS");
        const int v = e ? atoi(e) : 512;
        return v < 1 ? 1 : (v > 4096 ? 4096 : v);
    }();
    if (cap == 512) cap = ess_cap;
    int64_t g = (n + kScanBlock - 1) / kScanBlock;
    if (g > cap) g = cap;
    if (g < 1) g = 1;
    return (int)g;
}

void launch_aos_to_soa(smc_ctx *c, const double *aos, double *soa, int64_t n, int d, int64_t stride) {
    const int64_t tot = n * d;
    if (tot <= 0) return;
    hipLaunchKernelGGL(aos_to_soa_kernel, dim3((unsigned)((tot + 255) / 256)), dim3(256), 0, c->stream, aos, soa, n, d,
                       stride);
}
void launch_soa_to_aos(smc_ctx *c, const double *soa, double *aos, int64_t n, int d, int64_t stride) {
    const int64_t tot = n * d;
    if (tot <= 0) return;
    hipLaunchKernelGGL(soa_to_aos_kernel, dim3((unsigned)((tot + 255) / 256)), dim3(256), 0, c->stream, soa, aos, n, d,
                       stride);
}
void launch_sample_prior(smc_ctx *c, uint64_t seed, int64_t goff) {
    ParticleSet &P = c->set[SMC_SET_PRED];
    hipLaunchKernelGGL(sample_prior_kernel, dim3((unsigned)((c->n_local + 255) / 256)), dim3(256), 0, c->stream,
                       c->prior, P.theta, P.stride, c->n_local, seed, goff);
}
void launch_max(smc_ctx *c, const double *lk, int64_t n, double *d_out) {
    const int g = reduce_grid(n);
    hipLaunchKernelGGL(max_partial_kernel, dim3(g), dim3(kScanBlock), 0, c->stream, lk, n, c->d_partials);
    hipLaunchKernelGGL(max_final_kernel, dim3(1), dim3(kScanBlock), 0, c->stream, c->d_partials, g, d_out);
}
void launch_ess(smc_ctx *c, const double *lk, int64_t n, double max_lk, const double *gm, int k, double *d_out,
                const double *max_lk_dev) {
    EssCand cand{};
    cand.k = k;
    for (int i = 0; i < SMC_MAX_ESS_CAND; ++i) cand.gm[i] = (i < k) ? gm[i] : 0.0;
    const int g = reduce_grid(n, 512);
    int K;
    if (k <= 1) {
        K = 1;
        hipLaunchKernelGGL((ess_partial_kernel<1>), dim3(g), dim3(kScanBlock), 0, c->stream, lk, n, max_lk, max_lk_dev, cand,
                           c->d_partials);
    } else if (k <= 4) {
        K = 4;
        hipLaunchKernelGGL((ess_partial_kernel<4>), dim3(g), dim3(kScanBlock), 0, c->stream, lk, n, max_lk, max_lk_dev, cand,
                           c->d_partials);
    } else if (k <= 8) {
        K = 8;
        hipLaunchKernelGGL((ess_partial_kernel<8>), dim3(g), dim3(kScanBlock), 0, c->stream, lk, n, max_lk, max_lk_dev, cand,
                           c->d_partials);
    } else {
        K = 16;
        hipLaunchKernelGGL((ess_partial_kernel<16>), dim3(g), dim3(kScanBlock), 0, c->stream, lk, n, max_lk, max_lk_dev, cand,
                           c->d_partials);
    }
    hipLaunchKernelGGL(sum_rows_final_kernel, dim3(2 * K), dim3(kScanBlock), 0, c->stream, c->d_partials, g, 2 * K, d_out);
}
int ess_padded_k(int k) { return k <= 1 ? 1 : k <= 4 ? 4 : k <= 8 ? 8 : 16; }

void launch_moment_sums(smc_ctx *c, double *d_out) {
    ParticleSet &F = c->set[SMC_SET_FILT];
    const int g = reduce_grid(c->n_local);
    hipLaunchKernelGGL(moment_sum_kernel, dim3(g), dim3(kScanBlock), 0, c->stream, F.theta, F.stride, c->n_local,
                       c->dim, c->d_partials);
    hipLaunchKernelGGL(sum_rows_final_kernel, dim3(c->dim), dim3(kScanBlock), 0, c->stream, c->d_partials, g, c->dim, d_out);
}
void launch_moment_centered(smc_ctx *c, const double *mean, double *d_out) {
// ... 50 lines not shown
        }
        return;
    }
    if (v < nv) {
        double s = 0.0;
        for (int i = threadIdx.x; i < n_rows; i += blockDim.x) s += rows[(size_t)i * nv + v];
        s = block_sum(s, lds);
        if (threadIdx.x == 0) out[v] = s;
    } else if (threadIdx.x == 0) {
        out[nv] = (double)counters->accepted_now;
        out[nv + 1] = (double)counters->accepted_ever;
        out[nv + 2] = (double)counters->n_failed;
    }
}
void launch_moments_reduce(smc_ctx *c, int n_rows, int nv, double *d_out, const MHControl *ctl) {
    hipLaunchKernelGGL(moments_reduce_kernel, dim3(nv + 1), dim3(kScanBlock), 0, c->stream, c->d_partials, n_rows, nv, c->d_counters,
                       d_out, ctl, c->rank);
}

static ResampleArgs make_args(smc_ctx *c, double max_lk, double gm, double sum_w, double wrand, double base) {
    ResampleArgs a{};
    a.max_lk = max_lk;
    a.gm = gm;
    a.sum_w = sum_w;
    a.n_global = (double)c->n_global;
    a.inv_np = 1.0 / (double)c->n_global;
    a.wrand = wrand;
    a.base = base;
    a.first_rank = (c->rank == 0);
    a.scheme = c->resampling;
    a.thr = c->d_mn_thr;
    a.n_thr = c->n_global;
    a.s_full = 1.0 - ((double)c->n_global + 8.0) * 2.220446049250313e-16;
    return a;
}
void launch_resample_phase1(smc_ctx *c, double max_lk, double gm, double sum_w) {
    ParticleSet &P = c->set[SMC_SET_PRED];
    const ResampleArgs a = make_args(c, max_lk, gm, sum_w, 0.0, 0.0);
    const int64_t nt = c->n_tiles;
    hipLaunchKernelGGL(resample_tile_sums_kernel, dim3((unsigned)nt), dim3(kScanBlock), 0, c->stream, P.lk, c->n_local, a,
                       c->d_blk_r, c->d_blk_c);
    hipLaunchKernelGGL((tile_exclusive_scan_kernel<double>), dim3(1), dim3(kScanBlock), 0, c->stream, c->d_blk_r, nt);
    hipLaunchKernelGGL((tile_exclusive_scan_kernel<int64_t>), dim3(1), dim3(kScanBlock), 0, c->stream, c->d_blk_c, nt);
}
void launch_resample_phase2(smc_ctx *c, double max_lk, double gm, double sum_w, double base, double wrand) {
    ParticleSet &P = c->set[SMC_SET_PRED];
    const ResampleArgs a = make_args(c, max_lk, gm, sum_w, wrand, base);
    const int64_t nt = c->n_tiles;
    if (c->resampling == SMC_RESAMPLE_MULTINOMIAL) {
        const int64_t m = c->n_global + 1, ntm = (m + kScanTile - 1) / kScanTile;
        uint64_t seed;
        memcpy(&seed, &wrand, sizeof seed);
        hipLaunchKernelGGL(mn_spacings_kernel, dim3((unsigned)ntm), dim3(kScanBlock), 0, c->stream, seed,
                           0x5EEDull << 32, m, c->d_mn_thr, c->d_mn_blk);
        hipLaunchKernelGGL((tile_exclusive_scan_kernel<double>), dim3(1), dim3(kScanBlock), 0, c->stream, c->d_mn_blk, ntm);
        hipLaunchKernelGGL(mn_thresholds_kernel, dim3((unsigned)ntm), dim3(kScanBlock), 0, c->stream, m, c->d_mn_thr,
                           c->d_mn_blk, ntm);
    }
    hipLaunchKernelGGL(resample_offspring_kernel, dim3((unsigned)nt), dim3(kScanBlock), 0, c->stream, P.lk, c->n_local,
                       a, c->d_blk_r, c->d_oscan, c->d_blk_o);
    hipLaunchKernelGGL((tile_exclusive_scan_kernel<int64_t>), dim3(1), dim3(kScanBlock), 0, c->stream, c->d_blk_o, nt);
    hipLaunchKernelGGL(resample_apply_prefix_kernel, dim3((unsigned)nt), dim3(kScanBlock), 0, c->stream, c->d_oscan,
                       c->n_local, c->d_blk_o);
}
void launch_resample_gather_all(smc_ctx *c, int first_step, int64_t *d_result) {
    ParticleSet &P = c->set[SMC_SET_PRED];
    ParticleSet &F = c->set[SMC_SET_FILT];
    hipLaunchKernelGGL(resample_gather_all_kernel, dim3((unsigned)((c->n_local + 255) / 256)), dim3(256), 0, c->stream, c->d_oscan,
                       c->n_local, P.theta, P.stride, P.lk, c->dim, c->d_blk_c + c->n_tiles, c->d_blk_o + c->n_tiles, first_step,
                       F.theta, F.stride, F.lk, d_result);
}
void launch_offspring_from_scan(smc_ctx *c, int64_t *d_out) {
    hipLaunchKernelGGL(offspring_from_scan_kernel, dim3((unsigned)((c->n_local + 255) / 256)), dim3(256), 0, c->stream,
                       c->d_oscan, c->n_local, d_out);
}
void launch_resample_gather(smc_ctx *c, int64_t m_lo, int64_t m_hi, double *dst_theta, int64_t dst_stride,
                            double *dst_lk, int64_t dst_off) {
    const int64_t cnt = m_hi - m_lo;
    if (cnt <= 0) return;
    ParticleSet &P = c->set[SMC_SET_PRED];
    hipLaunchKernelGGL(resample_gather_kernel, dim3((unsigned)((cnt + 255) / 256)), dim3(256), 0, c->stream, c->d_oscan,
                       c->n_local, P.theta, P.stride, P.lk, c->dim, m_lo, m_hi, dst_theta, dst_stride, dst_lk, dst_off);
}
void launch_resample_stale(smc_ctx *c, int64_t lo, int64_t hi, int first_step) {
    if (hi <= lo) return;
    ParticleSet &P = c->set[SMC_SET_PRED];
    ParticleSet &F = c->set[SMC_SET_FILT];
    hipLaunchKernelGGL(resample_stale_rows_kernel, dim3((unsigned)((hi - lo + 255) / 256)), dim3(256), 0, c->stream,
                       P.theta, P.stride, P.lk, c->dim, lo, hi, first_step, F.theta, F.stride, F.lk);
}

}
```

python-based-sequential-monte-carlo-method-with-likelihood-tempering_amd/driver.py:

```python
from __future__ import annotations

import math
import time
from dataclasses import dataclass, field

import numpy as np

from .binding import SMC_MAX_ESS_CAND, SMC_SET_FILT, SMC_SET_PRED
from .comm import SingleComm
from .priors import sample_new_kind


@dataclass
class SMCSettings:
    n_particle: int = 1000
    ess_limit: float = 0.5
    mhstep_factor: float = 0.5
    mhstep_factor_cov: float = 0.5
    ad_mhstep_num: int = 20
    mhstep_num: int = 5
    r_threshold: float = 0.5
    r_threshold_f: float = 0.7
    r_threshold_min: float = 0.1
    d_gamma_max: float = 1
# ... 389 lines not shown
        wrand_u = np.random.rand() if rng == "numpy" else host_rng.rand()
        rs = resample(engine, comm, es, wrand_u, s, first_step=(step == 1), defer=s.defer_resample and not verbose)
        if verbose and rank == 0:
            log("n_tmp:", rs["n_tmp_before"])
        engine.reset_accept_flags()
        mhstep_ratio = 1.0
        if gamma_new >= 1.0:
            nMH, r_th = s.ad_mhstep_num, s.r_threshold_f
        else:
            nMH, r_th = s.mhstep_num, s.r_threshold
        j = 0
        acc_ever = 0
        mh_log = []
        fused = rng == "device" and _on_device(comm)
        batched = (fused and s.mh_batch not in (0, None) and getattr(engine, "mh_sweeps_device_rng", None) is not None
                   and getattr(engine, "model", ("",))[0] in ("mm", "methanation"))
        if batched:
            done, stopped = 0, False
            depth = s.mh_batch
            if depth == "auto":
                depth = (records[-1]["last_j"] + 1) if records else 2
            while done < nMH and not stopped:
                k = max(1, min(int(depth), nMH - done, 32))
                out = engine.mh_sweeps_device_rng(gamma_new, mhstep_ratio, w_cov, seed_device, (step << 16) | done, k,
                                                  r_th * n, s.r_threshold_min * n, lo)
                stats["mh_syncs"] += 1
                stats["mh_noop_sweeps"] += k - out["n_done"]
                for it in out["iterations"]:
                    account({"rk_attempts": it["rk_attempts"], "n_failed": 0}, it.get("counters"))
                    stats["rk_attempts_mh"] += it["rk_attempts"]
                    stats["mutation_sweeps"] += 1
                    stats["particle_mutation_steps"] += n
                    acc_ever = it["accepted_ever"]
                    mh_log.append({"cov_m": it["cov_m"], "mhstep_ratio": it["mhstep_ratio"], "accepted_now": it["accepted_now"],
                                   "accepted_ever": acc_ever})
                    if it["n_failed"]:
                        raise RuntimeError("an RK45 solve failed during an MH sweep (the reference raises here)")
                    if verbose and rank == 0:
                        if acc_ever > r_th * n:
                            log(f"r_ac.sum() > r_th * n_particle:{float(acc_ever)}")
                        elif acc_ever < s.r_threshold_min * n:
                            log(it["mhstep_ratio"] * 0.5)
                done += out["n_done"]
                stopped = out["stopped"]
                mhstep_ratio = out["ratio_next"]
                depth = 1 if s.mh_batch == "auto" else depth
            j = done - 1
        for j in ([] if batched else range(nMH)):
            stats["mh_syncs"] += 1
            if fused:
                out = engine.mh_iteration_device_rng(gamma_new, mhstep_ratio, w_cov, seed_device, (step << 16) | j, lo)
                cov_m = out["cov_m"]
                tot = [out["accepted_ever"], out["accepted_now"], out["n_failed"]]
                out = dict(out, n_failed=0)
            else:
                cov_m = proposal_cov(engine, comm, s, w_cov)
                if rng == "numpy":
                    noise = np.random.multivariate_normal(np.zeros(d), cov_m, n)
                    rr = np.random.uniform(0, 1, n)
                    out = engine.mh_step_host_rng(gamma_new, mhstep_ratio, noise[lo:lo + n_local], rr[lo:lo + n_local])
                else:
                    out = engine.mh_step_device_rng(gamma_new, mhstep_ratio, fix_row_signs(mvn_transform(cov_m)), seed_device,
                                                    (step << 16) | j, lo)
                tot = comm.allreduce_sum_i64([out["accepted_ever"], out["accepted_now"], out["n_failed"]])
            account(out)
            stats["rk_attempts_mh"] += out["rk_attempts"]
            stats["mutation_sweeps"] += 1
            stats["particle_mutation_steps"] += n
            acc_ever = int(tot[0])
            mh_log.append({"cov_m": cov_m, "mhstep_ratio": mhstep_ratio, "accepted_now": int(tot[1]),
                           "accepted_ever": acc_ever})
            if int(tot[2]):
                raise RuntimeError("an RK45 solve failed during an MH sweep (the reference raises here)")
            if acc_ever > r_th * n:
                if verbose and rank == 0:
                    log(f"r_ac.sum() > r_th * n_particle:{float(acc_ever)}")
                break
            if acc_ever < s.r_threshold_min * n:
                mhstep_ratio = mhstep_ratio * 0.5
                if verbose and rank == 0:
                    log(mhstep_ratio)
        if callable(rs):
            rs = rs()
        engine.commit_filt_to_pred()
        if verbose and rank == 0:
            log(f"iteration:{step}, nMH:{j}, Calculation time:{time.perf_counter() - start_time}, ESS:{ess}, "
                f"Max Likelihood:{max_lk}, New Gamma:{gamma_new}, Number of Adoption:{float(acc_ever)}")
        records.append({"step": step, "gamma_old": gamma_old, "gamma_new": gamma_new, "gm": es["gm"], "ess": ess,
                        "ess_iters": es["iters"], "sum_weight": es["sum_weight"], "max_lk": max_lk, "dlogZ": dlogZ,
                        "wrand_u": wrand_u, "last_j": j, "n_accept": float(acc_ever), "n_offspring": rs["n_offspring"],
                        "n_tmp_before": rs["n_tmp_before"], "mh": mh_log})
        if gamma_new == 1.0:
            break
        gamma_old = gamma_new
        if dump_dir:
            _dump(dump_dir, f"pred/{step}_p_pred", engine.download_particles(SMC_SET_PRED), rank, world)
            rst = np.random.get_state() if rng == "numpy" else host_rng.get_state()
            _save_state(dump_dir, step, rank, world, {"step": step, "gamma": gamma_new, "logZ": logZ, "rng": rng,
                                                      "n_particle": n, "rng_state": _rng_state_to_json(rst)})
    if gamma_new < 1.0 and verbose and rank == 0:
        log("tempering does't complete: last gamma =", gamma_new)
    engine.synchronize()
    if mm_shared0 is not None:
        stats["rk_attempts_shared"] = engine.share_info()["rk_attempts_shared"] - mm_shared0
    if mm_not_started0 is not None:
        stats["solves_not_started"] = engine.start_reject_info()["solves_not_started"] - mm_not_started0
    if dump_dir:
        final = engine.download_particles(SMC_SET_PRED)
        _dump(dump_dir, "pred/last_p_pred", final, rank, world)
        _dump(dump_dir, "Posterior_Distribution", final, rank, world, header=list(s.priors.keys()))
    pin = {"pinned": True} if (s.pinned_results and getattr(engine, "pinned_downloads", False)) else {}
    out = {"p_pred": engine.download_particles(SMC_SET_PRED, **pin), "lk": engine.download_lk(SMC_SET_PRED, **pin),
           "records": records, "logZ": logZ, "gamma": gamma_new, "step": step, "stats": stats,
           "wall_s": time.perf_counter() - start_time}
    if predictive is not None:
        out["predictive"] = engine.predictive_summary(**{"which": SMC_SET_PRED, "global_offset": lo, **predictive})
    if pointwise is not None and pointwise is not False:
        pw = {"which": SMC_SET_PRED, **(pointwise if isinstance(pointwise, dict) else {})}
        if pw.get("count_pit"):
            pw = {"global_offset": lo, **pw}
        out["pointwise"] = _pointwise_all_ranks(engine, comm, pw)
    return out
```

python-based-sequential-monte-carlo-method-with-likelihood-tempering_amd/engine.py:

```python
from __future__ import annotations

import ctypes

import numpy as np

from . import binding as B
from .binding import SMC_SET_FILT, SMC_SET_PRED, SmcError, check, lib


def _dp(a):
    return a.ctypes.data_as(B.c_dp)


def _f64(a, shape=None):
    a = np.ascontiguousarray(a, dtype=np.float64)
    if shape is not None and tuple(a.shape) != tuple(shape):
        raise ValueError(f"expected shape {shape}, got {a.shape}")
    return a


class _PinnedPool:

    def __init__(self, cap_bytes=1 << 30):
        import threading
# ... 322 lines not shown

    def set_share_replicates(self, enable=True):
        if "smc_set_share_replicates" in B.MISSING:
            return
        self._ck(self.L.smc_set_share_replicates(self.ctx, int(bool(enable))), "smc_set_share_replicates")

    def share_info(self):
        if "smc_mm_share_info" in B.MISSING:
            return {"n_solve": self.model[1], "rk_attempts_shared": 0}
        ns, sh = ctypes.c_int(0), ctypes.c_int64(0)
        self._ck(self.L.smc_mm_share_info(self.ctx, ctypes.byref(ns), ctypes.byref(sh)), "smc_mm_share_info")
        return {"n_solve": ns.value, "rk_attempts_shared": sh.value}

    def set_start_reject(self, enable=True):
        if "smc_set_start_reject" in B.MISSING:
            return
        self._ck(self.L.smc_set_start_reject(self.ctx, int(bool(enable))), "smc_set_start_reject")

    def start_reject_info(self):
        if "smc_mm_start_reject_info" in B.MISSING:
            return {"solves_not_started": 0}
        v = ctypes.c_int64(0)
        self._ck(self.L.smc_mm_start_reject_info(self.ctx, ctypes.byref(v)), "smc_mm_start_reject_info")
        return {"solves_not_started": v.value}

    def set_stiff_first(self, enable=True):
        if "smc_set_stiff_first" in B.MISSING:
            return
        self._ck(self.L.smc_set_stiff_first(self.ctx, int(bool(enable))), "smc_set_stiff_first")

    def set_resampling(self, scheme):
        k = B.RESAMPLING[scheme] if isinstance(scheme, str) else int(scheme)
        self._ck(self.L.smc_set_resampling(self.ctx, k), "smc_set_resampling")

    def upload_particles(self, which, aos):
        aos = _f64(aos)
        assert aos.ndim == 2 and aos.shape[1] == self.dim
        self._ck(self.L.smc_upload_particles(self.ctx, which, _dp(aos), aos.shape[0]), "smc_upload_particles")

    def download_particles(self, which, n=None, pinned=False):
        n = self.n_local if n is None else n
        out = pinned_empty((n, self.dim)) if pinned else np.empty((n, self.dim))
        self._ck(self.L.smc_download_particles(self.ctx, which, _dp(out), n), "smc_download_particles")
        return out

    def upload_lk(self, which, lk):
        lk = _f64(lk)
        self._ck(self.L.smc_upload_lk(self.ctx, which, _dp(lk), lk.shape[0]), "smc_upload_lk")

    def download_lk(self, which, n=None, pinned=False):
        n = self.n_local if n is None else n
        out = pinned_empty((n,)) if pinned else np.empty(n)
        self._ck(self.L.smc_download_lk(self.ctx, which, _dp(out), n), "smc_download_lk")
        return out

    def download_accept_flags(self):
        out = np.empty(self.n_local, dtype=np.uint8)
        self._ck(self.L.smc_download_accept_flags(self.ctx, out.ctypes.data_as(B.c_u8p), self.n_local),
                 "smc_download_accept_flags")
        return out

    def debug_set_order(self, order, patience=0):
        if order is None:
            self._ck(self.L.smc_debug_set_order(self.ctx, None, 0, 0), "smc_debug_set_order")
            return
        o = np.ascontiguousarray(order, dtype=np.int32)
        self._ck(self.L.smc_debug_set_order(self.ctx, o.ctypes.data_as(ctypes.POINTER(ctypes.c_int32)), o.size, int(patience)), "smc_debug_set_order")

    def download_item_info(self, n=None):
        n = self.n_local if n is None else int(n)
        out = np.empty((self.model[1], n), dtype=np.int32)
        self._ck(self.L.smc_download_item_info(self.ctx, out.ctypes.data_as(ctypes.POINTER(ctypes.c_int32)), n), "smc_download_item_info")
        return out

    def download_item_sums(self, n=None):
        n = self.n_local if n is None else int(n)
        out = np.empty((self.model[1], n), dtype=np.float64)
        self._ck(self.L.smc_download_item_sums(self.ctx, _dp(out), n), "smc_download_item_sums")
        return out

    def commit_filt_to_pred(self):
        self._ck(self.L.smc_commit_filt_to_pred(self.ctx), "smc_commit_filt_to_pred")

    def sample_prior_device(self, seed, global_offset=0):
        self._ck(self.L.smc_sample_prior_device(self.ctx, int(seed), int(global_offset)), "smc_sample_prior_device")

    def loglik(self, which=SMC_SET_PRED):
        nf, att = ctypes.c_int64(0), ctypes.c_int64(0)
        self._ck(self.L.smc_loglik(self.ctx, which, ctypes.byref(nf), ctypes.byref(att)), "smc_loglik")
        return {"n_failed": nf.value, "rk_attempts": att.value}

    def loglik_host(self, particle, want_pred=False):
        particle = _f64(particle)
        assert particle.ndim == 2 and particle.shape[1] == 3
        n = particle.shape[0]
        lk = np.empty(n)
        pred = np.empty((n, self.model[1], self.model[2])) if want_pred else None
        nf, att = ctypes.c_int64(0), ctypes.c_int64(0)
        self._ck(self.L.smc_mm_loglik_host(self.ctx, _dp(particle), n, _dp(lk), _dp(pred) if want_pred else None,
                                           ctypes.byref(nf), ctypes.byref(att)), "smc_mm_loglik_host")
        return lk, pred, {"n_failed": nf.value, "rk_attempts": att.value}

    def predict_user(self, particles):
        if self.model is None or self.model[0] != "user":
            raise SmcError("predict_user: no user model has been set")
        particles = _f64(particles)
        if particles.ndim != 2 or particles.shape[1] != self.dim:
            raise ValueError(f"predict_user: particles must be (n, {self.dim}), got {particles.shape}")
        n = particles.shape[0]
        lk = np.empty(n)
        pred = np.empty((n, self.model[1], self.model[2], self.user_n_obs))
        nf, att = ctypes.c_int64(0), ctypes.c_int64(0)
        self._ck(self.L.smc_user_predict(self.ctx, _dp(particles), n, _dp(lk), _dp(pred), ctypes.byref(nf), ctypes.byref(att)),
                 "smc_user_predict")
        return lk, pred, {"n_failed": nf.value, "rk_attempts": att.value}

    def _design(self, what, t, cond, inputs=None, events=None):
        if t is None:
            if cond is not None or inputs is not None or events is not None:
                raise ValueError(f"{what}: cond, inputs or events without t (a design is all of them, or none for the data's own)")
            return None, None, (None, None, 0, 0), (self.model[1], self.model[2])
        from .user_models import design_layout
        t = _f64(t)
        design_layout(t, cond, self.user_n_cond)
        if inputs is not None:
            if self.user_n_in == 0:
                raise ValueError(f"{what}: inputs for a model that has none")
            in_t, in_u, n_in = self._inputs(what, inputs, t.shape[0])
            if n_in != self.user_n_in:
                raise ValueError(f"{what}: the model has {self.user_n_in} inputs, the design's u holds {n_in}")
            self._ck(self.L.smc_user_set_design_inputs(self.ctx, _dp(in_t), _dp(in_u), t.shape[0], in_t.shape[1]),
                     "smc_user_set_design_inputs")
        elif self.user_n_in:
            self._ck(self.L.smc_user_set_design_inputs(self.ctx, None, None, 0, 0), "smc_user_set_design_inputs")
        if events is not None:
            if self.user_n_ev == 0:
                raise ValueError(f"{what}: events for a model that has none")
            ev_t, ev_v, n_val = self._events(what, events, t)
            if n_val != self.user_n_val:
                raise ValueError(f"{what}: the model's events hold {self.user_n_val} values, the design's hold {n_val}")
            if ev_t.shape[1] > self.user_n_ev:
                raise ValueError(f"{what}: the model was compiled for {self.user_n_ev} events per row, the design's rows hold {ev_t.shape[1]}")
            self._ck(self.L.smc_user_set_design_events(self.ctx, _dp(ev_t), None if ev_v is None else _dp(ev_v), t.shape[0], ev_t.shape[1]),
                     "smc_user_set_design_events")
        elif self.user_n_ev:
            self._ck(self.L.smc_user_set_design_events(self.ctx, None, None, 0, 0), "smc_user_set_design_events")
        cond = np.zeros((t.shape[0], 0)) if cond is None else _f64(np.asarray(cond, dtype=np.float64).reshape(t.shape[0], -1))
        cbuf = np.ascontiguousarray(cond if cond.size else np.zeros((t.shape[0], 1)))
        return t, cbuf, (_dp(t), _dp(cbuf), t.shape[0], t.shape[1]), t.shape

    def predict_user_at(self, particles, t=None, cond=None, inputs=None, events=None):
        if self.model is None or self.model[0] != "user":
            raise SmcError("predict_user_at: no user model has been set")
        particles = _f64(particles)
        if particles.ndim != 2 or particles.shape[1] != self.dim:
            raise ValueError(f"predict_user_at: particles must be (n, {self.dim}), got {particles.shape}")
        t, cbuf, cargs, shape = self._design("predict_user_at", t, cond, inputs, events)
        n = particles.shape[0]
        pred = np.empty((n, shape[0], shape[1], self.user_n_obs))
        nf, att = ctypes.c_int64(0), ctypes.c_int64(0)
        self._ck(self.L.smc_user_predict_at(self.ctx, _dp(particles), n, *cargs, _dp(pred), ctypes.byref(nf), ctypes.byref(att)),
                 "smc_user_predict_at")
        return pred, {"n_failed": nf.value, "rk_attempts": att.value}

    def predictive_summary(self, which=SMC_SET_FILT, probs=(0.025, 0.5, 0.975), t=None, cond=None, noise=False, seed=0,
                           global_offset=0, max_staging_bytes=0, inputs=None, events=None):
# ... 318 lines not shown
```

Before: 483.6 million.

## Chain per-step reductions and resample on device, swap particle sets instead of copying

Adds a single-rank 'step chain' path. It fuses the max-lk final reduction into the ESS partial kernel, chains the moment sums, centered moments and MH control into device-only kernels, and runs resampling as tile sums, scan, offspring, prefix and a gather that also clears accept flags. The filtered set is committed to predicted by swapping pointers instead of doing device-to-device copies, and the separate accept-flag memset is skipped when the gather already cleared it. The aim is fewer kernel launches, fewer host-side phases and less copy traffic per tempering step, at the cost of more code paths and state flags that must stay consistent.

```diff
diff --git a/include/smc_hip.h b/include/smc_hip.h
--- a/include/smc_hip.h
+++ b/include/smc_hip.h
@@ -202,6 +202,10 @@
 int smc_download_item_info(smc_ctx *ctx, int32_t *info, int64_t n);
 int smc_download_item_sums(smc_ctx *ctx, double *sums, int64_t n);
 int smc_commit_filt_to_pred(smc_ctx *ctx);
+int smc_set_step_chain(smc_ctx *ctx, int enable);
+int smc_step_chain_info(smc_ctx *ctx, int *active, int *scan_block, int *scan_tile, int *reduce_blocks, int *ess_blocks);
+int smc_commit_swap(smc_ctx *ctx);
+int smc_debug_download_resample_scan(smc_ctx *ctx, double *blk_r, int32_t *oscan);
 int smc_sample_prior_device(smc_ctx *ctx, uint64_t seed, int64_t global_offset);
 
 int smc_loglik(smc_ctx *ctx, int set, int64_t *n_failed, int64_t *rk_attempts);
diff --git a/python-based-sequential-monte-carlo-method-with-likelihood-tempering_amd/binding.py b/python-based-sequential-monte-carlo-method-with-likelihood-tempering_amd/binding.py
--- a/python-based-sequential-monte-carlo-method-with-likelihood-tempering_amd/binding.py
+++ b/python-based-sequential-monte-carlo-method-with-likelihood-tempering_amd/binding.py
@@ -160,6 +160,10 @@
     "smc_download_item_sums": (cint, [c_ctx, c_dp, i64]),
     "smc_debug_set_order": (cint, [c_ctx, ctypes.POINTER(ctypes.c_int32), i64, cint]),
     "smc_commit_filt_to_pred": (cint, [c_ctx]),
+    "smc_set_step_chain": (cint, [c_ctx, cint]),
+    "smc_step_chain_info": (cint, [c_ctx, c_ip, c_ip, c_ip, c_ip, c_ip]),
+    "smc_commit_swap": (cint, [c_ctx]),
+    "smc_debug_download_resample_scan": (cint, [c_ctx, c_dp, ctypes.POINTER(ctypes.c_int32)]),
     "smc_sample_prior_device": (cint, [c_ctx, u64, i64]),
     "smc_loglik": (cint, [c_ctx, cint, c_i64p, c_i64p]),
     "smc_mm_loglik_host": (cint, [c_ctx, c_dp, i64, c_dp, c_dp, c_i64p, c_i64p]),
diff --git a/python-based-sequential-monte-carlo-method-with-likelihood-tempering_amd/csrc/smc_api.hip b/python-based-sequential-monte-carlo-method-with-likelihood-tempering_amd/csrc/smc_api.hip
--- a/python-based-sequential-monte-carlo-method-with-likelihood-tempering_amd/csrc/smc_api.hip
+++ b/python-based-sequential-monte-carlo-method-with-likelihood-tempering_amd/csrc/smc_api.hip
@@ -10,6 +10,7 @@
 #include <cstring>
 #include <mutex>
 #include <new>
+#include <utility>
 
 #include "exchange_plan.h"
 #include "replicate_groups.h"
@@ -179,6 +180,8 @@
         c->share_env_off = e ? atoi(e) == 0 : false;
         e = getenv("SMC_START_REJECT");
         c->start_reject_env_off = e ? atoi(e) == 0 : false;
+        e = getenv("SMC_STEP_CHAIN");
+        c->step_chain_env_off = e ? atoi(e) == 0 : false;
     }
 #define CK(call)                                   \
     do {                                           \
@@ -226,7 +229,7 @@
     c->d_rr = c->d_noise + (size_t)n_local * dim;
     CK(hipMalloc(&c->d_stage, nb * dim));
     c->partials_cap = 2048 * 64;
-    CK(hipMalloc(&c->d_partials, (size_t)c->partials_cap * sizeof(double)));
+    CK(hipMalloc(&c->d_partials, (size_t)(c->partials_cap + 2048) * sizeof(double)));
     CK(hipMalloc(&c->d_small, 4096 * sizeof(double)));
     {
         BatchBlock *db = nullptr, *hb = nullptr;
@@ -752,6 +755,7 @@
 int smc_reset_accept_flags(smc_ctx *c) {
     if (!c) return fail(nullptr, "NULL context");
     HIPC(c, hipSetDevice(c->device));
+    if (c->r_ac_zero) return 0;
     HIPC(c, hipMemsetAsync(c->r_ac, 0, (size_t)c->n_local, c->stream));
     return 0;
 }
@@ -763,6 +767,37 @@
     HIPC(c, hipMemcpyAsync(c->set[SMC_SET_PRED].theta, c->set[SMC_SET_FILT].theta, nb * c->dim,
                            hipMemcpyDeviceToDevice, c->stream));
     HIPC(c, hipMemcpyAsync(c->set[SMC_SET_PRED].lk, c->set[SMC_SET_FILT].lk, nb, hipMemcpyDeviceToDevice, c->stream));
+    return 0;
+}
+static bool chain_on(const smc_ctx *c) { return c->step_chain && !c->step_chain_env_off && c->world == 1 && !can_reduce(c); }
+int smc_set_step_chain(smc_ctx *c, int enable) {
+    if (!c) return fail(nullptr, "NULL context");
+    c->step_chain = enable ? 1 : 0;
+    return 0;
+}
+int smc_step_chain_info(smc_ctx *c, int *active, int *scan_block, int *scan_tile, int *reduce_blocks, int *ess_blocks) {
+    if (!c) return fail(nullptr, "NULL context");
+    if (active) *active = chain_on(c) ? 1 : 0;
+    if (scan_block) *scan_block = kScanBlock;
+    if (scan_tile) *scan_tile = kScanTile;
+    if (reduce_blocks) *reduce_blocks = 2048;
+    if (ess_blocks) *ess_blocks = 512;
+    return 0;
+}
+int smc_commit_swap(smc_ctx *c) {
+    if (!c) return fail(nullptr, "NULL context");
+    if (!chain_on(c)) return smc_commit_filt_to_pred(c);
+    c->ess_max_valid = false;
+    c->moments_valid = false;
+    std::swap(c->set[SMC_SET_PRED], c->set[SMC_SET_FILT]);
+    return 0;
+}
+int smc_debug_download_resample_scan(smc_ctx *c, double *blk_r, int32_t *oscan) {
+    if (!c) return fail(nullptr, "NULL context");
+    HIPC(c, hipSetDevice(c->device));
+    if (blk_r) HIPC(c, hipMemcpyAsync(blk_r, c->d_blk_r, (size_t)(c->n_tiles + 1) * sizeof(double), hipMemcpyDeviceToHost, c->stream));
+    if (oscan) HIPC(c, hipMemcpyAsync(oscan, c->d_oscan, (size_t)c->n_local * sizeof(int32_t), hipMemcpyDeviceToHost, c->stream));
+    HIPC(c, hipStreamSynchronize(c->stream));
     return 0;
 }
 int smc_sample_prior_device(smc_ctx *c, uint64_t seed, int64_t global_offset) {
@@ -996,25 +1031,30 @@
     HIPC(c, hipSetDevice(c->device));
     constexpr int kMaxAt = 0, kSumsAt = 8;
     double *S = c->d_ess;
-    if (with_max) {
+    const int n_a = n_cand < SMC_MAX_ESS_CAND ? n_cand : SMC_MAX_ESS_CAND, n_b = n_cand - n_a;
+    const int pad_a = ess_padded_k(n_a), pad_b = n_b > 0 ? ess_padded_k(n_b) : 0;
+    const int nv = 2 * (pad_a + pad_b);
+    if (!with_max && !c->ess_max_valid)
+        return fail(c, "smc_ess_search_global: with_max == 0 needs an earlier call with with_max != 0 on the same lk");
+    bool chained = false;
+    if (chain_on(c)) {
+        chained = launch_ess_search_chain(c, c->set[SMC_SET_PRED].lk, c->n_local, gm, n_a, n_b, with_max, S + kMaxAt, S + kSumsAt);
+        if (chained && with_max) c->ess_max_valid = true;
+    }
+    if (!chained && with_max) {
         {
             ScopedTimer tm(c, SMC_T_MAX);
             launch_max(c, c->set[SMC_SET_PRED].lk, c->n_local, S + kMaxAt);
         }
         if (dev_allreduce(c, S + kMaxAt, 1, ncclDouble, ncclMax)) return 1;
         c->ess_max_valid = true;
-    } else if (!c->ess_max_valid) {
-        return fail(c, "smc_ess_search_global: with_max == 0 needs an earlier call with with_max != 0 on the same lk");
-    }
-    const int n_a = n_cand < SMC_MAX_ESS_CAND ? n_cand : SMC_MAX_ESS_CAND, n_b = n_cand - n_a;
-    const int pad_a = ess_padded_k(n_a), pad_b = n_b > 0 ? ess_padded_k(n_b) : 0;
-    {
+    }
+    if (!chained) {
         ScopedTimer tm(c, SMC_T_ESS);
         launch_ess(c, c->set[SMC_SET_PRED].lk, c->n_local, 0.0, gm, n_a, S + kSumsAt, S + kMaxAt);
         if (n_b > 0) launch_ess(c, c->set[SMC_SET_PRED].lk, c->n_local, 0.0, gm + n_a, n_b, S + kSumsAt + 2 * pad_a, S + kMaxAt);
     }
     HIPC(c, hipGetLastError());
-    const int nv = 2 * (pad_a + pad_b);
     if (dev_allreduce(c, S + kSumsAt, (size_t)nv, ncclDouble, ncclSum)) return 1;
     HIPC(c, hipMemcpyAsync(c->h_ess + kMaxAt, S + kMaxAt, (size_t)(kSumsAt - kMaxAt + nv) * sizeof(double), hipMemcpyDeviceToHost,
                            c->stream));
@@ -1081,7 +1121,11 @@
         return 0;
     }
     c->moments_valid = false;
-    {
+    if (chain_on(c)) {
+        ScopedTimer tm(c, SMC_T_RESAMPLE);
+        launch_resample_chain(c, max_lk, gm, sum_weight_global, wrand, first_step, c->d_rs);
+        c->r_ac_zero = true;
+    } else {
         ScopedTimer tm(c, SMC_T_RESAMPLE);
         launch_resample_phase1(c, max_lk, gm, sum_weight_global);
         launch_resample_phase2(c, max_lk, gm, sum_weight_global, 0.0, wrand);
@@ -1440,6 +1484,7 @@
     mh.pratio = c->d_pratio;
     {
         ScopedTimer tm(c, SMC_T_MH);
+        c->r_ac_zero = false;
         if (c->model_kind == 2) launch_meth_mh(c, n, mh); else if (c->model_kind == 3) launch_user_mh(c, n, mh); else launch_mm_mh(c, n, mh);
     }
     return mh_finish(c, accepted_now, accepted_ever, n_failed, rk_attempts);
@@ -1465,6 +1510,7 @@
     for (int i = 0; i < c->dim * c->dim; ++i) mh.transform[i] = transform[i];
     {
         ScopedTimer tm(c, SMC_T_MH);
+        c->r_ac_zero = false;
         if (c->model_kind == 2) launch_meth_mh(c, c->n_local, mh); else if (c->model_kind == 3) launch_user_mh(c, c->n_local, mh); else launch_mm_mh(c, c->n_local, mh);
     }
     return mh_finish(c, accepted_now, accepted_ever, n_failed, rk_attempts);
@@ -1527,6 +1573,7 @@
     }
     {
         ScopedTimer tm(c, SMC_T_MH);
+        c->r_ac_zero = false;
         if (c->model_kind == 2) launch_meth_mh(c, c->n_local, mh); else if (c->model_kind == 3) launch_user_mh(c, c->n_local, mh); else launch_mm_mh(c, c->n_local, mh);
     }
     HIPC(c, hipGetLastError());
@@ -1599,14 +1646,20 @@
         if (mm && c->moments_valid) {
             a.mom = S + kV;
             a.sums = nullptr;
+            launch_mh_control(c, a, w_cov);
+        } else if (chain_on(c)) {
+            a.mom = S + kCent;
+            a.sums = S + kSums;
+            launch_moments_control_chain(c, S + kSums, S + kCent, a, w_cov);
         } else {
             if (two_pass(0)) return bail();
             a.mom = S + kCent;
             a.sums = S + kSums;
+            launch_mh_control(c, a, w_cov);
         }
-        launch_mh_control(c, a, w_cov);
     }
     c->moments_valid = false;
+    c->r_ac_zero = false;
     for (int i = 0; i < n_iter; ++i) {
         MHParams mh{};
         mh.gamma = gamma;
diff --git a/python-based-sequential-monte-carlo-method-with-likelihood-tempering_amd/csrc/smc_internal.h b/python-based-sequential-monte-carlo-method-with-likelihood-tempering_amd/csrc/smc_internal.h
--- a/python-based-sequential-monte-carlo-method-with-likelihood-tempering_amd/csrc/smc_internal.h
+++ b/python-based-sequential-monte-carlo-method-with-likelihood-tempering_amd/csrc/smc_internal.h
@@ -256,6 +256,9 @@
     int n_solve = 0, partner_mask = 0;
     int groups[2 * smc::kMaxEx]{};
     int *d_groups = nullptr;
+    int step_chain = 1;
+    bool step_chain_env_off = false;
+    bool r_ac_zero = false;
     int exact_pow = 0;
     bool solve_lds_raised = false;
     int cu_count = 0, solve_blocks_per_cu = 0, solve_blocks_per_cu_fast = 0;
diff --git a/python-based-sequential-monte-carlo-method-with-likelihood-tempering_amd/csrc/stage_kernels.h b/python-based-sequential-monte-carlo-method-with-likelihood-tempering_amd/csrc/stage_kernels.h
--- a/python-based-sequential-monte-carlo-method-with-likelihood-tempering_amd/csrc/stage_kernels.h
+++ b/python-based-sequential-monte-carlo-method-with-likelihood-tempering_amd/csrc/stage_kernels.h
@@ -23,4 +23,8 @@
                             double *dst_lk, int64_t dst_off);
 void launch_resample_stale(smc_ctx *c, int64_t lo, int64_t hi, int first_step);
 void launch_resample_gather_all(smc_ctx *c, int first_step, int64_t *d_result);
+bool launch_ess_search_chain(smc_ctx *c, const double *lk, int64_t n, const double *gm, int n_a, int n_b, int with_max,
+                             double *d_max, double *d_sums);
+void launch_moments_control_chain(smc_ctx *c, double *d_sums, double *d_cent, const MHControlArgs &a, const double *w_cov);
+void launch_resample_chain(smc_ctx *c, double max_lk, double gm, double sum_w, double wrand, int first_step, int64_t *d_result);
 }
diff --git a/python-based-sequential-monte-carlo-method-with-likelihood-tempering_amd/csrc/stage_kernels.hip b/python-based-sequential-monte-carlo-method-with-likelihood-tempering_amd/csrc/stage_kernels.hip
--- a/python-based-sequential-monte-carlo-method-with-likelihood-tempering_amd/csrc/stage_kernels.hip
+++ b/python-based-sequential-monte-carlo-method-with-likelihood-tempering_amd/csrc/stage_kernels.hip
@@ -111,9 +111,7 @@
         partials[blockIdx.x] = r;
     }
 }
-__global__ void __launch_bounds__(kScanBlock) max_final_kernel(const double *__restrict__ partials, int np,
-                                                               double *__restrict__ out) {
-    __shared__ double lds[4];
+__device__ __forceinline__ double max_rows_value(const double *__restrict__ partials, int np, double *lds ) {
     double m = -__longlong_as_double(0x7ff0000000000000LL);
     for (int i = threadIdx.x; i < np; i += blockDim.x) {
         const double v = partials[i];
@@ -123,11 +121,15 @@
     const int w = threadIdx.x >> 6, l = threadIdx.x & 63;
     if (l == 0) lds[w] = m;
     __syncthreads();
-    if (threadIdx.x == 0) {
-        double r = lds[0];
-        for (int i = 1; i < 4; ++i) r = (lds[i] > r || lds[i] != lds[i]) ? lds[i] : r;
-        out[0] = r;
-    }
+    double r = lds[0];
+    for (int i = 1; i < 4; ++i) r = (lds[i] > r || lds[i] != lds[i]) ? lds[i] : r;
+    return r;
+}
+__global__ void __launch_bounds__(kScanBlock) max_final_kernel(const double *__restrict__ partials, int np,
+                                                               double *__restrict__ out) {
+    __shared__ double lds[4];
+    const double r = max_rows_value(partials, np, lds);
+    if (threadIdx.x == 0) out[0] = r;
 }
 
 struct EssCand {
@@ -160,10 +162,8 @@
 }
 
 template <int K>
-__global__ void __launch_bounds__(kScanBlock) ess_partial_kernel(const double *__restrict__ lk, int64_t n, double max_lk_val,
-                                                                 const double *__restrict__ max_lk_dev, EssCand cand,
-                                                                 double *__restrict__ partials) {
-    const double max_lk = max_lk_dev ? *max_lk_dev : max_lk_val;
+__device__ __forceinline__ void ess_partial_body(const double *__restrict__ lk, int64_t n, const double max_lk, const EssCand &cand,
+                                                 double *__restrict__ partials) {
     constexpr int NV = 2 * K;
     constexpr int kShift = NV == 2 ? 5 : NV == 8 ? 3 : NV == 16 ? 2 : 1;
     static_assert(NV == 2 || NV == 8 || NV == 16 || NV == 32, "K must be 1, 4, 8 or 16");
@@ -190,15 +190,74 @@
         partials[(size_t)blockIdx.x * NV + threadIdx.x] = r;
     }
 }
+template <int K>
+__global__ void __launch_bounds__(kScanBlock) ess_partial_kernel(const double *__restrict__ lk, int64_t n, double max_lk_val,
+                                                                 const double *__restrict__ max_lk_dev, EssCand cand,
+                                                                 double *__restrict__ partials) {
+    const double max_lk = max_lk_dev ? *max_lk_dev : max_lk_val;
+    ess_partial_body<K>(lk, n, max_lk, cand, partials);
+}
+template <int K>
+__global__ void __launch_bounds__(kScanBlock) ess_partial_chain_kernel(const double *__restrict__ lk, int64_t n,
+                                                                       const double *__restrict__ max_partials, int np_max,
+                                                                       double *__restrict__ max_out, EssCand cand,
+                                                                       double *__restrict__ partials) {
+    __shared__ double lds[4];
+    __shared__ double s_max;
+    const double r = max_rows_value(max_partials, np_max, lds);
+    if (threadIdx.x == 0) {
+        s_max = r;
+        if (blockIdx.x == 0) max_out[0] = r;
+    }
+    __syncthreads();
+    ess_partial_body<K>(lk, n, s_max, cand, partials);
+}
+template <int NV>
+__device__ __forceinline__ double sum_rows_values(const double *__restrict__ partials, int np, int nvals, int v0, int nv,
+                                                  double (*wpart)[NV] ) {
+    double acc[NV];
+#pragma unroll
+    for (int k = 0; k < NV; ++k) acc[k] = 0.0;
+    for (int i = threadIdx.x; i < np; i += blockDim.x) {
+        const double *row = partials + (size_t)i * nvals + v0;
+#pragma unroll
+        for (int k = 0; k < NV; ++k)
+            if (k < nv) acc[k] += row[k];
+    }
+    __syncthreads();
+#pragma unroll
+    for (int k = 0; k < NV; ++k) {
+        const double ws = wave_sum(acc[k]);
+        if ((threadIdx.x & 63) == 0) wpart[threadIdx.x >> 6][k] = ws;
+    }
+    __syncthreads();
+    double r = 0.0;
+    if ((int)threadIdx.x < nv) {
+        r = wpart[0][threadIdx.x];
+        for (int q = 1; q < (int)(blockDim.x >> 6); ++q) r += wpart[q][threadIdx.x];
+    }
+    return r;
+}
+__device__ __forceinline__ double sum_rows_value(const double *__restrict__ partials, int np, int nvals, int v,
+                                                 double (*wpart)[1]) {
+    return sum_rows_values<1>(partials, np, nvals, v, 1, wpart);
+}
 __global__ void __launch_bounds__(kScanBlock) sum_rows_final_kernel(const double *__restrict__ partials, int np,
                                                                     int nvals, double *__restrict__ out) {
-    __shared__ double lds[4];
+    __shared__ double lds[kScanBlock / 64][1];
     for (int v = blockIdx.x; v < nvals; v += gridDim.x) {
-        double s = 0.0;
-        for (int i = threadIdx.x; i < np; i += blockDim.x) s += partials[(size_t)i * nvals + v];
-        s = block_sum(s, lds);
+        const double s = sum_rows_value(partials, np, nvals, v, lds);
         if (threadIdx.x == 0) out[v] = s;
     }
+}
+__global__ void __launch_bounds__(kScanBlock) sum_rows_final_pair_kernel(const double *__restrict__ rows_a, int nv_a,
+                                                                         const double *__restrict__ rows_b, int nv_b, int np,
+                                                                         double *__restrict__ out) {
+    __shared__ double lds[kScanBlock / 64][1];
+    const int v = blockIdx.x;
+    if (v >= nv_a + nv_b) return;
+    const double s = v < nv_a ? sum_rows_value(rows_a, np, nv_a, v, lds) : sum_rows_value(rows_b, np, nv_b, v - nv_a, lds);
+    if (threadIdx.x == 0) out[v] = s;
 }
 
 __global__ void __launch_bounds__(kScanBlock) moment_sum_kernel(const double *__restrict__ theta, int64_t stride,
@@ -216,16 +275,10 @@
 struct MeanArg {
     double m[SMC_MAX_DIM];
 };
-__global__ void __launch_bounds__(kScanBlock) moment_centered_kernel(const double *__restrict__ theta, int64_t stride,
-                                                                     int64_t n, int d, MeanArg mean,
-                                                                     const double *__restrict__ dev_sums, double n_div,
-                                                                     double *__restrict__ partials) {
-    __shared__ double lds[4];
-    __shared__ double s_mu[SMC_MAX_DIM];
+__device__ __forceinline__ void moment_centered_body(const double *__restrict__ theta, int64_t stride, int64_t n, int d,
+                                                     const double *s_mu, double *lds, double *__restrict__ partials) {
     double acc[SMC_MAX_DIM * (SMC_MAX_DIM + 1) / 2];
     const int npair = d * (d + 1) / 2;
-    if ((int)threadIdx.x < d) s_mu[threadIdx.x] = dev_sums ? dev_sums[threadIdx.x] / n_div : mean.m[threadIdx.x];
-    __syncthreads();
     for (int k = 0; k < npair; ++k) acc[k] = 0.0;
     for (int64_t i = (int64_t)blockIdx.x * blockDim.x + threadIdx.x; i < n; i += (int64_t)gridDim.x * blockDim.x) {
         double x[SMC_MAX_DIM];
@@ -239,6 +292,31 @@
         if (threadIdx.x == 0) partials[(size_t)blockIdx.x * npair + k] = s;
     }
 }
+__global__ void __launch_bounds__(kScanBlock) moment_centered_kernel(const double *__restrict__ theta, int64_t stride,
+                                                                     int64_t n, int d, MeanArg mean,
+                                                                     const double *__restrict__ dev_sums, double n_div,
+                                                                     double *__restrict__ partials) {
+    __shared__ double lds[4];
+    __shared__ double s_mu[SMC_MAX_DIM];
+    if ((int)threadIdx.x < d) s_mu[threadIdx.x] = dev_sums ? dev_sums[threadIdx.x] / n_div : mean.m[threadIdx.x];
+    __syncthreads();
+    moment_centered_body(theta, stride, n, d, s_mu, lds, partials);
+}
+__global__ void __launch_bounds__(kScanBlock) moment_centered_chain_kernel(const double *__restrict__ theta, int64_t stride,
+                                                                           int64_t n, int d, const double *__restrict__ sum_rows,
+                                                                           int np, double n_div, double *__restrict__ sums_out,
+                                                                           double *__restrict__ partials) {
+    __shared__ double lds[4];
+    __shared__ double wpart[kScanBlock / 64][SMC_MAX_DIM];
+    __shared__ double s_mu[SMC_MAX_DIM];
+    const double s = sum_rows_values<SMC_MAX_DIM>(sum_rows, np, d, 0, d, wpart);
+    if ((int)threadIdx.x < d) {
+        s_mu[threadIdx.x] = s / n_div;
+        if (blockIdx.x == 0) sums_out[threadIdx.x] = s;
+    }
+    __syncthreads();
+    moment_centered_body(theta, stride, n, d, s_mu, lds, partials);
+}
 
 template <int D>
 __global__ void mh_transform_kernel(const double *__restrict__ mom, const double *__restrict__ sums, double n_global, WCov wcov,
@@ -251,6 +329,20 @@
 template <int D>
 __global__ void __launch_bounds__(kScanBlock) mh_control_kernel(MHControlArgs a, WCov wcov) {
     __shared__ double wpart[kScanBlock / 64][D + D * (D + 1) / 2];
+    mh_control_body<D, false>(a, wcov, wpart);
+}
+template <int D>
+__global__ void __launch_bounds__(kScanBlock) mh_control_chain_kernel(MHControlArgs a, WCov wcov, const double *__restrict__ cent_rows,
+                                                                      int np, double *cent_out) {
+    __shared__ double wpart[kScanBlock / 64][D + D * (D + 1) / 2];
+    constexpr int npair = D * (D + 1) / 2;
+    __shared__ double cpart[kScanBlock / 64][npair];
+    __shared__ double s_cent[npair];
+    const double s = sum_rows_values<npair>(cent_rows, np, npair, 0, npair, cpart);
+    if ((int)threadIdx.x < npair) s_cent[threadIdx.x] = s;
+    __syncthreads();
+    if (threadIdx.x == 0)
+        for (int k = 0; k < npair; ++k) cent_out[k] = s_cent[k];
     mh_control_body<D, false>(a, wcov, wpart);
 }
 
@@ -452,6 +544,28 @@
         if (i < n) oscan[i] += off;
     }
 }
+__global__ void __launch_bounds__(kScanBlock) resample_apply_prefix_chain_kernel(int32_t *__restrict__ oscan, int64_t n,
+                                                                                 int64_t *blk_o, int64_t *blk_c, int64_t nt) {
+    const int64_t base = ((int64_t)blockIdx.x * kScanBlock + threadIdx.x) * kScanItems;
+    __shared__ int64_t lds[4];
+    const int64_t b = blockIdx.x;
+    int64_t s = 0;
+    for (int64_t j = threadIdx.x; j < b; j += kScanBlock) s += blk_o[j];
+    const int64_t below = block_sum(s, lds);
+    if (b == nt - 1 && threadIdx.x == 0) blk_o[nt] = below + blk_o[b];
+    if (b == 0) {
+        int64_t cs = 0;
+        for (int64_t j = threadIdx.x; j < nt; j += kScanBlock) cs += blk_c[j];
+        cs = block_sum(cs, lds);
+        if (threadIdx.x == 0) blk_c[nt] = cs;
+    }
+    const int32_t off = (int32_t)below;
+#pragma unroll
+    for (int k = 0; k < kScanItems; ++k) {
+        const int64_t i = base + k;
+        if (i < n) oscan[i] += off;
+    }
+}
 
 __global__ void offspring_from_scan_kernel(const int32_t *__restrict__ oscan, int64_t n, int64_t *__restrict__ p_is) {
     const int64_t i = (int64_t)blockIdx.x * blockDim.x + threadIdx.x;
@@ -479,11 +593,13 @@
     dst_lk[dst_off + k] = src_lk[j];
 }
 
-__global__ void __launch_bounds__(256)
-resample_gather_all_kernel(const int32_t *__restrict__ oscan, int64_t n, const double *__restrict__ src_theta, int64_t src_stride,
-                           const double *__restrict__ src_lk, int d, const int64_t *__restrict__ count_total,
-                           const int64_t *__restrict__ offspring_total, int first_step, double *__restrict__ dst_theta,
-                           int64_t dst_stride, double *__restrict__ dst_lk, int64_t *__restrict__ result ) {
+template <bool CLEAR_FLAGS>
+__device__ __forceinline__ void
+resample_gather_all_body(const int32_t *__restrict__ oscan, int64_t n, const double *__restrict__ src_theta, int64_t src_stride,
+                         const double *__restrict__ src_lk, int d, const int64_t *__restrict__ count_total,
+                         const int64_t *__restrict__ offspring_total, int first_step, double *__restrict__ dst_theta,
+                         int64_t dst_stride, double *__restrict__ dst_lk, int64_t *__restrict__ result ,
+                         uint8_t *__restrict__ r_ac) {
     const int64_t m = (int64_t)blockIdx.x * blockDim.x + threadIdx.x;
     const int64_t total = *offspring_total;
     if (m == 0) {
@@ -491,6 +607,7 @@
         result[1] = total;
     }
     if (m >= n) return;
+    if constexpr (CLEAR_FLAGS) r_ac[m] = 0;
     if (m < total) {
         int64_t lo = 0, hi = n;
         while (lo < hi) {
@@ -507,6 +624,23 @@
         for (int c = 0; c < d; ++c) dst_theta[c * dst_stride + m] = first_step ? 0.0 : src_theta[c * src_stride + m];
         dst_lk[m] = first_step ? 0.0 : src_lk[m];
     }
+}
+__global__ void __launch_bounds__(256)
+resample_gather_all_kernel(const int32_t *__restrict__ oscan, int64_t n, const double *__restrict__ src_theta, int64_t src_stride,
+                           const double *__restrict__ src_lk, int d, const int64_t *__restrict__ count_total,
+                           const int64_t *__restrict__ offspring_total, int first_step, double *__restrict__ dst_theta,
+                           int64_t dst_stride, double *__restrict__ dst_lk, int64_t *__restrict__ result ) {
+    resample_gather_all_body<false>(oscan, n, src_theta, src_stride, src_lk, d, count_total, offspring_total, first_step, dst_theta,
+                                    dst_stride, dst_lk, result, nullptr);
+}
+__global__ void __launch_bounds__(256)
+resample_gather_all_clear_kernel(const int32_t *__restrict__ oscan, int64_t n, const double *__restrict__ src_theta,
+                                 int64_t src_stride, const double *__restrict__ src_lk, int d,
+                                 const int64_t *__restrict__ count_total, const int64_t *__restrict__ offspring_total, int first_step,
+                                 double *__restrict__ dst_theta, int64_t dst_stride, double *__restrict__ dst_lk,
+                                 int64_t *__restrict__ result , uint8_t *__restrict__ r_ac) {
+    resample_gather_all_body<true>(oscan, n, src_theta, src_stride, src_lk, d, count_total, offspring_total, first_step, dst_theta,
+                                   dst_stride, dst_lk, result, r_ac);
 }
 
 __global__ void resample_stale_rows_kernel(const double *__restrict__ src_theta, int64_t src_stride,
@@ -723,6 +857,91 @@
     hipLaunchKernelGGL(resample_gather_kernel, dim3((unsigned)((cnt + 255) / 256)), dim3(256), 0, c->stream, c->d_oscan,
                        c->n_local, P.theta, P.stride, P.lk, c->dim, m_lo, m_hi, dst_theta, dst_stride, dst_lk, dst_off);
 }
+static_assert(2048 * (SMC_MAX_DIM + SMC_MAX_DIM * (SMC_MAX_DIM + 1) / 2) <= 2048 * 64, "d_partials holds both sets of moment rows");
+static inline double *chain_max_rows(smc_ctx *c) { return c->d_partials + c->partials_cap; }
+static inline double *chain_centered_rows(smc_ctx *c) { return c->d_partials + 2048 * SMC_MAX_DIM; }
+
+template <bool CHAIN>
+static void launch_ess_rows(smc_ctx *c, const double *lk, int64_t n, const double *gm, int k, int g, double *rows,
+                            const double *max_dev, const double *max_rows, int np_max, double *max_out) {
+    EssCand cand{};
+    cand.k = k;
+    for (int i = 0; i < SMC_MAX_ESS_CAND; ++i) cand.gm[i] = (i < k) ? gm[i] : 0.0;
+#define SMC_ESS(K)                                                                                                              \
+    do {                                                                                                                        \
+        if (CHAIN)                                                                                                              \
+            hipLaunchKernelGGL((ess_partial_chain_kernel<K>), dim3(g), dim3(kScanBlock), 0, c->stream, lk, n, max_rows, np_max,  \
+                               max_out, cand, rows);                                                                            \
+        else                                                                                                                    \
+            hipLaunchKernelGGL((ess_partial_kernel<K>), dim3(g), dim3(kScanBlock), 0, c->stream, lk, n, 0.0, max_dev, cand,      \
+                               rows);                                                                                           \
+    } while (0)
+    if (k <= 1) SMC_ESS(1); else if (k <= 4) SMC_ESS(4); else if (k <= 8) SMC_ESS(8); else SMC_ESS(16);
+#undef SMC_ESS
+}
+bool launch_ess_search_chain(smc_ctx *c, const double *lk, int64_t n, const double *gm, int n_a, int n_b, int with_max,
+                             double *d_max, double *d_sums) {
+    const int g = reduce_grid(n, 512), g_max = reduce_grid(n);
+    const int pad_a = ess_padded_k(n_a), pad_b = n_b > 0 ? ess_padded_k(n_b) : 0;
+    if ((int64_t)g * 2 * (pad_a + pad_b) > c->partials_cap) return false;
+    double *rows_a = c->d_partials, *rows_b = c->d_partials + (size_t)g * 2 * pad_a;
+    if (with_max) {
+        ScopedTimer tm(c, SMC_T_MAX);
+        hipLaunchKernelGGL(max_partial_kernel, dim3(g_max), dim3(kScanBlock), 0, c->stream, lk, n, chain_max_rows(c));
+    }
+    ScopedTimer tm(c, SMC_T_ESS);
+    if (with_max) {
+        launch_ess_rows<true>(c, lk, n, gm, n_a, g, rows_a, nullptr, chain_max_rows(c), g_max, d_max);
+    } else {
+        launch_ess_rows<false>(c, lk, n, gm, n_a, g, rows_a, d_max, nullptr, 0, nullptr);
+    }
+    if (n_b > 0) launch_ess_rows<false>(c, lk, n, gm + n_a, n_b, g, rows_b, d_max, nullptr, 0, nullptr);
+    hipLaunchKernelGGL(sum_rows_final_pair_kernel, dim3(2 * (pad_a + pad_b)), dim3(kScanBlock), 0, c->stream, rows_a, 2 * pad_a,
+                       rows_b, 2 * pad_b, g, d_sums);
+    return true;
+}
+void launch_moments_control_chain(smc_ctx *c, double *d_sums, double *d_cent, const MHControlArgs &a, const double *w_cov) {
+    ParticleSet &F = c->set[SMC_SET_FILT];
+    const int g = reduce_grid(c->n_local);
+    hipLaunchKernelGGL(moment_sum_kernel, dim3(g), dim3(kScanBlock), 0, c->stream, F.theta, F.stride, c->n_local, c->dim,
+                       c->d_partials);
+    hipLaunchKernelGGL(moment_centered_chain_kernel, dim3(g), dim3(kScanBlock), 0, c->stream, F.theta, F.stride, c->n_local,
+                       c->dim, c->d_partials, g, (double)c->n_global, d_sums, chain_centered_rows(c));
+    WCov w{};
+    for (int i = 0; i < c->dim * c->dim; ++i) w.w[i] = w_cov[i];
+#define SMC_CT(D) case D: hipLaunchKernelGGL((mh_control_chain_kernel<D>), dim3(1), dim3(kScanBlock), 0, c->stream, a, w, \
+                                             chain_centered_rows(c), g, d_cent); break
+    switch (c->dim) {
+        SMC_CT(1); SMC_CT(2); SMC_CT(3); SMC_CT(4); SMC_CT(5); SMC_CT(6); SMC_CT(7); SMC_CT(8);
+    }
+#undef SMC_CT
+}
+void launch_resample_chain(smc_ctx *c, double max_lk, double gm, double sum_w, double wrand, int first_step, int64_t *d_result) {
+    ParticleSet &P = c->set[SMC_SET_PRED];
+    ParticleSet &F = c->set[SMC_SET_FILT];
+    const ResampleArgs a = make_args(c, max_lk, gm, sum_w, wrand, 0.0);
+    const int64_t nt = c->n_tiles;
+    hipLaunchKernelGGL(resample_tile_sums_kernel, dim3((unsigned)nt), dim3(kScanBlock), 0, c->stream, P.lk, c->n_local, a,
+                       c->d_blk_r, c->d_blk_c);
+    hipLaunchKernelGGL((tile_exclusive_scan_kernel<double>), dim3(1), dim3(kScanBlock), 0, c->stream, c->d_blk_r, nt);
+    if (c->resampling == SMC_RESAMPLE_MULTINOMIAL) {
+        const int64_t m = c->n_global + 1, ntm = (m + kScanTile - 1) / kScanTile;
+        uint64_t seed;
+        memcpy(&seed, &wrand, sizeof seed);
+        hipLaunchKernelGGL(mn_spacings_kernel, dim3((unsigned)ntm), dim3(kScanBlock), 0, c->stream, seed,
+                           0x5EEDull << 32, m, c->d_mn_thr, c->d_mn_blk);
+        hipLaunchKernelGGL((tile_exclusive_scan_kernel<double>), dim3(1), dim3(kScanBlock), 0, c->stream, c->d_mn_blk, ntm);
+        hipLaunchKernelGGL(mn_thresholds_kernel, dim3((unsigned)ntm), dim3(kScanBlock), 0, c->stream, m, c->d_mn_thr,
+                           c->d_mn_blk, ntm);
+    }
+    hipLaunchKernelGGL(resample_offspring_kernel, dim3((unsigned)nt), dim3(kScanBlock), 0, c->stream, P.lk, c->n_local,
+                       a, c->d_blk_r, c->d_oscan, c->d_blk_o);
+    hipLaunchKernelGGL(resample_apply_prefix_chain_kernel, dim3((unsigned)nt), dim3(kScanBlock), 0, c->stream, c->d_oscan,
+                       c->n_local, c->d_blk_o, c->d_blk_c, nt);
+    hipLaunchKernelGGL(resample_gather_all_clear_kernel, dim3((unsigned)((c->n_local + 255) / 256)), dim3(256), 0, c->stream,
+                       c->d_oscan, c->n_local, P.theta, P.stride, P.lk, c->dim, c->d_blk_c + nt, c->d_blk_o + nt, first_step,
+                       F.theta, F.stride, F.lk, d_result, c->r_ac);
+}
 void launch_resample_stale(smc_ctx *c, int64_t lo, int64_t hi, int first_step) {
     if (hi <= lo) return;
     ParticleSet &P = c->set[SMC_SET_PRED];
diff --git a/python-based-sequential-monte-carlo-method-with-likelihood-tempering_amd/driver.py b/python-based-sequential-monte-carlo-method-with-likelihood-tempering_amd/driver.py
--- a/python-based-sequential-monte-carlo-method-with-likelihood-tempering_amd/driver.py
+++ b/python-based-sequential-monte-carlo-method-with-likelihood-tempering_amd/driver.py
@@ -495,7 +495,10 @@
                     log(mhstep_ratio)
         if callable(rs):
             rs = rs()
-        engine.commit_filt_to_pred()
+        if world == 1 and gamma_new < 1.0 and step + 1 < s.itr_max and getattr(engine, "commit_swap", None) is not None:
+            engine.commit_swap()
+        else:
+            engine.commit_filt_to_pred()
         if verbose and rank == 0:
             log(f"iteration:{step}, nMH:{j}, Calculation time:{time.perf_counter() - start_time}, ESS:{ess}, "
                 f"Max Likelihood:{max_lk}, New Gamma:{gamma_new}, Number of Adoption:{float(acc_ever)}")
diff --git a/python-based-sequential-monte-carlo-method-with-likelihood-tempering_amd/engine.py b/python-based-sequential-monte-carlo-method-with-likelihood-tempering_amd/engine.py
--- a/python-based-sequential-monte-carlo-method-with-likelihood-tempering_amd/engine.py
+++ b/python-based-sequential-monte-carlo-method-with-likelihood-tempering_amd/engine.py
@@ -428,6 +428,30 @@
     def commit_filt_to_pred(self):
         self._ck(self.L.smc_commit_filt_to_pred(self.ctx), "smc_commit_filt_to_pred")
 
+    def commit_swap(self):
+        if "smc_commit_swap" in B.MISSING:
+            return self.commit_filt_to_pred()
+        self._ck(self.L.smc_commit_swap(self.ctx), "smc_commit_swap")
+
+    def set_step_chain(self, enable=True):
+        if "smc_set_step_chain" in B.MISSING:
+            return
+        self._ck(self.L.smc_set_step_chain(self.ctx, int(bool(enable))), "smc_set_step_chain")
+
+    def step_chain_info(self):
+        v = [ctypes.c_int(0) for _ in range(5)]
+        self._ck(self.L.smc_step_chain_info(self.ctx, *[ctypes.byref(x) for x in v]), "smc_step_chain_info")
+        return dict(zip(("active", "scan_block", "scan_tile", "reduce_blocks", "ess_blocks"), (x.value for x in v)))
+
+    def debug_resample_scan(self):
+        tile = self.step_chain_info()["scan_tile"]
+        blk_r = np.empty((self.n_local + tile - 1) // tile + 1, dtype=np.float64)
+        oscan = np.empty(self.n_local, dtype=np.int32)
+        self._ck(self.L.smc_debug_download_resample_scan(self.ctx, blk_r.ctypes.data_as(B.c_dp),
+                                                         oscan.ctypes.data_as(ctypes.POINTER(ctypes.c_int32))),
+                 "smc_debug_download_resample_scan")
+        return blk_r, oscan
+
     def sample_prior_device(self, seed, global_offset=0):
         self._ck(self.L.smc_sample_prior_device(self.ctx, int(seed), int(global_offset)), "smc_sample_prior_device")
 
```

After: 483.4 million (median of 2 runs). No clear change (-0.1%).
